# cmbant/getdist

Measured on AMD Instinct MI355X. Metric: 2D KDE densities/sec (triangle, 50 params, 1e+07 samples), higher is better.
Workload: dtype f64

## Files before the change

getdist_amd/_lib.py:

```python

import ctypes as C
import os
import subprocess

import numpy as np

_HERE = os.path.dirname(os.path.abspath(__file__))
LIB_PATH = os.path.join(_HERE, "csrc", "libgdhip.so")

GD_OK, GD_ERR_BADARG, GD_ERR_NOMEM, GD_ERR_HIP, GD_ERR_EMPTY, GD_ERR_SOLVER, GD_ERR_FFT, GD_ERR_NODEVICE, GD_ERR_TIMEOUT = \
    0, -1, -2, -3, -4, -5, -6, -7, -8


class GdhipError(RuntimeError):
    def __init__(self, code, msg):
        super().__init__("libgdhip error %d: %s" % (code, msg))
        self.code = code


class GdhipTimeout(GdhipError):
    """GD_ERR_TIMEOUT: a collective or the communicator set-up gave up waiting for a peer; the library has aborted and dropped
    the communicator, so the ranks renegotiate over the host application's own channel (parallel.init_library_comm)."""


# ... 35 lines not shown
    "gd_kde_lag_sums_2d": (C.c_int, [_p, _i32, _i32, _pd, _pi64, _i32, _pd]),
    "gd_autocov_lags_batch": (C.c_int, [_p, _pi32, _i32, _pd, _i64, _i32, _pd]),
    "gd_kde_lag_sums_batch": (C.c_int, [_p, _pi32, _i32, _pd, _pi64, _i32, _pd]),
    "gd_autocov_lags_range_batch": (C.c_int, [_p, _pi32, _i32, _pd, _i64, _i64, _i64, _i32, _pd]),
    "gd_timer_start": (C.c_int, [_p]),
    "gd_timer_stop_ms": (C.c_int, [_p, _pd]),
    "gd_upload": (C.c_int, [_p, _p, _i64, _i64, _i64, _i64, _p]),
    "gd_num_rows": (C.c_int, [_p, _pi64, _pi64]),
    "gd_column_ptr": (C.c_int, [_p, _i64, C.POINTER(_p)]),
    "gd_weight_stats": (C.c_int, [_p, _i64, _i64, _f64, _pd]),
    "gd_col_stats": (C.c_int, [_p, _i64, _i64, _pd]),
    "gd_cov": (C.c_int, [_p, _pi32, _i32, _i64, _i64, _pd, _pd, _pd, _pd]),
    "gd_quantiles": (C.c_int, [_p, _pi32, _i32, _i64, _i64, _pd, _i32, _pd]),
    "gd_quantiles_mm_probe": (C.c_int, [_p, _pi32, _i32, _i64, _i64, _pd, _i32, _pd, _pd, _pd, _pd, C.POINTER(C.c_int32)]),
    "gd_quantiles_mm": (C.c_int, [_p, _pi32, _i32, _i64, _i64, _pd, _i32, _pd, _pd]),
    "gd_autocov_lags": (C.c_int, [_p, _i32, _f64, _i64, _i32, _pd]),
    "gd_kde_lag_sums": (C.c_int, [_p, _i32, _f64, _pi64, _i32, _pd]),
    "gd_hist1d": (C.c_int, [_p, _pi32, _i32, _pd, _pd, _i32, _pd]),
    "gd_hist1d_dev": (C.c_int, [_p, _pi32, _i32, _pd, _pd, _i32, _p]),
    "gd_bin_indices": (C.c_int, [_p, _i32, _f64, _f64, _i32, _i32, _pi32, _pi64]),
    "gd_prebin": (C.c_int, [_p, _i32, _f64, _f64, _i32, _p]),
    "gd_prebin_batch": (C.c_int, [_p, _pi32, _i32, _pd, _pd, _i32, C.POINTER(_p)]),
    "gd_prebin8_batch": (C.c_int, [_p, _pi32, _i32, _pd, _pd, _i32, C.POINTER(_p), _pi64]),
    "gd_hist2d_prebinned8": (C.c_int, [_p, _i32, C.POINTER(_p), C.POINTER(_p), _p]),
    "gd_prebin8_hist2d": (C.c_int, [_p, _pi32, _i32, _pd, _pd, C.POINTER(_p), _pi64, _i32, C.POINTER(_p), C.POINTER(_p), _p]),
    "gd_hist2d": (C.c_int, [_p, _i32, _pi32, _pi32, _pd, _pd, _pd, _pd, _i32, _p]),
    "gd_hist2d_prebinned": (C.c_int, [_p, _i32, C.POINTER(_p), C.POINTER(_p), _i32, _p]),
    "gd_minmax_affine": (C.c_int, [_p, _i32, _pi32, _pi32, _pd, _pd, _pd]),
    "gd_hist2d_sheared": (C.c_int, [_p, _i32, _pi32, _pi32, _pd, _pd, _pd, _pd, _pd, _pd, _i32, _p]),
    "gd_dct1d": (C.c_int, [_p, _i32, _i32, _pd, _pd]),
    "gd_isj1d": (C.c_int, [_p, _i32, _i32, _pd, _pd, _pd, _pi32]),
    "gd_isj1d_dev": (C.c_int, [_p, _i32, _i32, _p, _pd, _pd, _pi32]),
    "gd_density1d": (C.c_int, [_p, _i32, _i32, _pd, _pd, _pi32, _pi32, _i32, _i32, _pd, _pi32]),
    "gd_density1d_dev": (C.c_int, [_p, _i32, _i32, _p, _pd, _pi32, _pi32, _i32, _i32, _pd, _pi32]),
    "gd_density1d_batch": (C.c_int, [_p, _p, _p, _i32, _pi32, _i32, _pd, _pd, _pd]),
    "gd_kopt2d": (C.c_int, [_p, _i32, _i32, _p, _pd, _pi32, _pd, _pd, _pd]),
    "gd_kopt2d_enqueue": (C.c_int, [_p, _i32, _i32, _p, _pd, _pi32, _pd, _pd, _p, _pi32]),
    "gd_kopt2d_finish": (C.c_int, [_p, _p, _i32, _i32, _p, _pd]),
    "gd_get_h": (C.c_int, [_p, _i32, _pd, _pd, _pd, _pi32, _pd]),
    "gd_density2d": (C.c_int, [_p, _i32, _i32, _p, _pd, _pd, _pd, _pi32, _pi32, _i32, _i32, _p, _pi32]),
    "gd_copy_mark": (C.c_int, [_p, _pi32]),
    "gd_copy_wait": (C.c_int, [_p, _i32]),
    "gd_density2d_enqueue": (C.c_int, [_p, _i32, _i32, _p, _pd, _pd, _pd, _pi32, _pi32, _i32, _i32, _p, _p]),
    "gd_density2d_enqueue_indexed": (C.c_int, [_p, _i32, _i32, _p, _pi32, _pd, _pd, _pd, _pi32, _pi32, _i32, _i32, _p, _p]),
    "gd_attach_samples": (C.c_int, [_p, _p]),
    "gd_clone_samples": (C.c_int, [_p, _p]),
    "gd_bind_thread": (C.c_int, [_p]),
    "gd_contour_levels": (C.c_int, [_p, _i32, _i32, _p, _pd, _i32, _pd, _pi32]),
    "gd_contour_paths": (C.c_int, [_p, _i32, _p, _pi64, _pi32, _pi32, _pd, _pi64, _i64, _pd, _pi64, _i64, _pd, _i32, _p, _p, _pi64,
                                   _pi64, _pi32]),
    "gd_limits1d": (C.c_int, [_p, _i32, _i32, _pd, _pd, _pd, _pd, _i32, _i32, _pd, _pi32]),
    "gd_set_extra_column": (C.c_int, [_p, _i32, _pd]),
    "gd_aux_weights": (C.c_int, [_p, _pd]),
    "gd_col_minmax": (C.c_int, [_p, _pi32, _i32, _i64, _i64, _i32, C.c_double, _pd]),
    "gd_weights_integral": (C.c_int, [_p, _pi32]),
    "gd_thin_rows": (C.c_int, [_p, _i64, _i64, _i64, _i32, _p, _i64, C.POINTER(C.c_int64)]),
    "gd_binary_transitions": (C.c_int, [_p, _pi32, _i32, _p, _i64, _pd, _i32, C.POINTER(C.c_int64)]),
    "gd_thinned_lag_sums": (C.c_int, [_p, _pi32, _i32, _pd, _p, _i64, _i32, _pd]),
    "gd_density2d_masked": (C.c_int, [_p, _i32, _p, C.c_double, C.c_double, C.c_double, _i32, _i32, _i32, _i32, _pd, _pd,
                                      C.POINTER(C.c_ubyte), _p, _pi32]),
    "gd_like_weights": (C.c_int, [_p, _pd, _i32, C.c_double, _pd]),
    "gd_select_weights": (C.c_int, [_p, _i32]),
    "gd_likes1d": (C.c_int, [_p, _i32, _i32, _pd, _pd, _pd, _pd, _pi32, _pi32, _i32, _pd, _pi32]),
    "gd_likes2d": (C.c_int, [_p, _i32, _i32, _p, _p, _pd, _pd, _pd, _pi32, _pi32, _i32, _p, _pi32]),
    "gd_circ_convolve": (C.c_int, [_p, _i32, _i32, _pd, _pd, _pd]),
    "gd_convolve1d_direct": (C.c_int, [_p, _pd, _i64, _pd, _i64, _pd]),
    "gd_autoconvolve": (C.c_int, [_p, _i32, _f64, _i32, _pd, _i64, _i64, _i64, _i32, _pd]),
    "gd_like_stats": (C.c_int, [_p, _i32, _pd]),
    "gd_batch2d_grid_sizes": (C.c_int, [_p, _i32, _pd, _pi32, _i32, _pi32]),
    "gd_density2d_batch": (C.c_int, [_p, _p, _p, _p, _i32, _pd, _pd, _pd, _pi32, _i32, _p, _p, _p, _i64, _pi32, _pd, _pd, _pi32,
                                     _pi32]),
    "gd_comm_unique_id": (C.c_int, [_p]),
    "gd_comm_init": (C.c_int, [_p, _i32, _i32, _p]),
    "gd_comm_info": (C.c_int, [_p, _pi32, _pi32]),
    "gd_comm_destroy": (C.c_int, [_p]),
    "gd_comm_abandon": (C.c_int, [_p]),
    "gd_comm_allgather": (C.c_int, [_p, _pd, _i64, _pd]),
    "gd_comm_allreduce_sum": (C.c_int, [_p, _pd, _i64]),
    "gd_comm_allgather_dev": (C.c_int, [_p, _p, _i64, _p]),
    "gd_comm_allreduce_sum_dev": (C.c_int, [_p, _p, _i64, _p]),
    "gd_batch2d_finish": (C.c_int, [_p]),
    "gd_batch2d_invalidate": (C.c_int, [_p]),
    "gd_batch2d_exchanges": (C.c_int, [_p, C.POINTER(C.c_int64)]),
    "gd_comm_rccl_path": (C.c_int, [C.c_char_p, C.c_int32, C.POINTER(C.c_int32)]),
    "gd_upload_shard": (C.c_int, [_p, _p, _i64, _i64, _i64, _i64, _i64, _p]),
    "gd_comm_share_columns": (C.c_int, [_p, C.POINTER(C.c_int64)]),
    "gd_histnd_batch": (C.c_int, [_p, _i32, _pi32, _pi32, _pd, _pd, _i32, _i32, _i32, _pd, _pd, _pd]),
    "gd_pca_corr": (C.c_int, [_p, _pi32, _i32, _pi32, _pd, _pd, _pd]),
    "gd_pca_project": (C.c_int, [_p, _pi32, _i32, _pi32, _pd, _pd, _pd, _i32, _i32, _pd, _pd, _pd, _pd, _pd, _pd]),
    "gd_mixture_nll": (C.c_int, [_p, _pi32, _i32, _i32, _pd, _pd, _pd, _i64, _i64, _pd]),
    "gd_draw_single_rows": (C.c_int, [_p, C.POINTER(C.c_uint64), _p, _f64, _f64, _i32, _p, _i64, _pi64]),
    "gd_gather_rows": (C.c_int, [_p, _p, _i64, _pi32, _i32, _p]),
    "gd_format_rows": (C.c_int, [_p, _pi32, _i32, _i64, _i64, _p, _i64, _i32, _i32, _i32, _i32, _p, _i64, _pi64]),
    "gd_format_matrix": (C.c_int, [_p, _p, _i64, _i32, _i64, _i64, _i32, _i32, _i32, _i32, _p, _i64, _pi64]),
    "gd_parse_scan": (C.c_int, [_p, _p, _i64, _i32, _pi64, _pi32, _pi64]),
    "gd_parse_rows": (C.c_int, [_p, _p, _i64, _i32, _i64, _i32, _p, _i64, _i64, _p, _i64, _pi64]),
    "gd_expr_eval": (C.c_int, [_p, _pi32, _i32, _pd, _i32, _i32, _i32, _i64, _i64, _p, _pd]),
    "gd_expr_eval_tab": (C.c_int, [_p, _pi32, _i32, _pd, _i32, _i32, _i32, _i64, _i64, _p, _pd, _p, _i32]),
    "gd_upload_device": (C.c_int, [_p, _p, _i32, _i32, _i32, _pi32, _i32, C.POINTER(_p), _i32]),
    "gd_pointer_info": (C.c_int, [_p, _p, _pi32, _pi32]),
    "gd_fetch_device_array": (C.c_int, [_p, _p, _i64, _i64, _i64, _i64, _i32, _p, _pd]),
    "gd_download_samples": (C.c_int, [_p, _pd]),
    "gd_select_samples": (C.c_int, [_p, _p, _pi64]),
    "gd_set_weights": (C.c_int, [_p, _pd]),
    "gd_export_device": (C.c_int, [_p, _p, _pi64]),
    "gd_export_alloc": (C.c_int, [_i32, _i64, C.POINTER(_p)]),
    "gd_export_free": (C.c_int, [_i32, _p]),
    "gd_export_fetch": (C.c_int, [_i32, _p, _p, _i64]),
}

GD_HISTND_MAXD, GD_HISTND_MAX_BINS = 25, 1 << 25
GD_HISTND_H, GD_HISTND_LIKES, GD_HISTND_LMIN = 1, 2, 4
GD_PCA_MAX_PROJ = 448
GD_DRAW_MORE_ROWS = -21
GD_FORMAT_MORE_BYTES = -22
GD_FMT_SRC_WEIGHT, GD_FMT_SRC_ZERO, GD_FMT_SRC_ONE = -1, -2, -3
GD_FMT_MAX_PREC, GD_FMT_MAX_WIDTH = 17, 32
GD_PARSE_NOT_PLAIN = -23
GD_ERR_DECLINED, GD_ERR_OTHER_DEVICE, GD_ERR_NOT_DEVICE = -24, -25, -26
GD_PTR_DEVICE, GD_PTR_PINNED, GD_PTR_MANAGED, GD_PTR_UNKNOWN = 0, 1, 2, 3
GD_PARSE_MAX_LINE = 8192
GD_EX_MAX_CODE, GD_EX_MAX_STACK, GD_EX_MAX_CONST, GD_EX_MAX_COLS = 128, 16, 32, 16
GD_EX_WEIGHT = -1
GD_EX_OPS = ("COL CONST NEG ABS SQRT SQUARE RECIP EXP LOG LOG10 LOG2 SIN COS TAN ATAN TANH NOT ADD SUB MUL DIV POW ATAN2 MIN MAX "
             "LT LE GT GE EQ NE AND OR WHERE").split()
GD_EX_TO_COLUMN, GD_EX_TO_AUXW, GD_EX_TO_HOST_F64, GD_EX_TO_HOST_U8 = 0, 1, 2, 3
GD_TAB_OPS = {"INTERP": 34, "SPLINE1": 35, "SPLINE2": 36}
GD_TAB_MAX_TABLES, GD_TAB_MAX_DOUBLES = 4, 1 << 22
GD_PATHS_XY, GD_PATHS_FLAG, GD_PATHS_LOOPS = 0, 1, 2
PATHS_ALLOC_FN = C.CFUNCTYPE(C.c_void_p, C.c_void_p, _i32, _i64)


class GdExprTable(C.Structure):

    _fields_ = [("kind", _i32), ("deriv", _i32), ("nx", _i32), ("ny", _i32), ("p0", _pd), ("p1", _pd), ("p2", _pd),
                ("left", _f64), ("right", _f64)]


def expr_table_structs(tables):
    arr = (GdExprTable * len(tables))()
    for t, st in zip(tables, arr):
        st.kind, st.deriv, st.nx, st.ny = GD_TAB_OPS[t.kind], t.deriv, t.nx, t.ny
        for name, a in zip(("p0", "p1", "p2"), t.arrays):
            setattr(st, name, _dp(a))
        st.left, st.right = t.left, t.right
    return arr


def format_field_bytes(width, prec):
    return max(int(width), int(prec) + 8) + 1


def skipped_text_bytes(f, skiprows):
    start = 0
    for _ in range(int(skiprows or 0)):
        line = f.readline()
        if not line:
            break
        if b"\r" in line.replace(b"\r\n", b"") or b"\0" in line or not line.isascii():
            return None
        start += len(line)
    return start


class GdDevPart(C.Structure):

    _fields_ = [("base", _p), ("rows", _i64), ("cols", _i64), ("row_stride", _i64), ("col_stride", _i64), ("weights", _p),
                ("w_stride", _i64)]


class GdSelection(C.Structure):

    _fields_ = [("row_kind", _i32), ("flags", _i32), ("lo", _i64), ("hi", _i64), ("rows", _p), ("K", _i64), ("thr", _f64),
                ("keep", _p), ("m", _i32), ("append_kind", _i32), ("append_slot", _i32), ("weight_kind", _i32),
                ("append_host", _p), ("new_weights", _p)]


class GdExport(C.Structure):

    _fields_ = [("row_kind", _i32), ("flags", _i32), ("lo", _i64), ("hi", _i64), ("rows", _p), ("K", _i64), ("thr", _f64),
                ("mask_col", _i32), ("m", _i32), ("cols", _p), ("base", _p), ("rows_capacity", _i64), ("row_stride", _i64),
                ("col_stride", _i64), ("dtype", _i32), ("reserved", _i32), ("consumer_stream", _p)]


GD_EXP_ROWS_COLUMN_NZ = 5

GD_SEL_ALL, GD_SEL_RANGE, GD_SEL_MASK_U8, GD_SEL_WEIGHT_GT, GD_SEL_ROWS_I32 = range(5)
GD_SEL_W_KEEP, GD_SEL_W_UNIT, GD_SEL_W_REPLACE = range(3)
GD_SEL_APPEND_NONE, GD_SEL_APPEND_HOST, GD_SEL_APPEND_SLOT = range(3)
GD_SEL_ROWS_ON_DEVICE = 1
GD_SEL_TILE = 1024

_lib = None


def load_library():
    global _lib
    if _lib is None:
        if not os.path.exists(LIB_PATH):
            raise ImportError("libgdhip.so is not built: run `python -c 'import __graft_entry__ as g; g.build()'` "
                              "or getdist_amd/csrc/build.sh (there is no CPU fallback)")
        lib = C.CDLL(LIB_PATH)
        for name, (res, args) in SIGNATURES.items():
            fn = getattr(lib, name)
            fn.restype = res
            fn.argtypes = args
        _lib = lib
    return _lib


def _dp(a):
    return a.ctypes.data_as(_pd)


def _ip(a):
    return a.ctypes.data_as(_pi32)


def _f64arr(a):
    return np.ascontiguousarray(a, dtype=np.float64)


def _i32arr(a):
    return np.ascontiguousarray(a, dtype=np.int32)


class DevBuf:

    def __init__(self, ctx, nbytes):
        self.ctx = ctx
        self.nbytes = int(nbytes)
        self.ptr, self.capacity = ctx._take_block(self.nbytes)

    def free(self):
        if self.ptr and self.ctx.h:
            self.ctx._give_block(self.ptr, self.capacity)
        self.ptr = None

    def __del__(self):
        try:
            self.free()
        except Exception:
            pass

    def to_host(self, shape, dtype=np.float64, offset_bytes=0, pinned=False):
        out = self.ctx.pinned_array(shape, dtype) if pinned else np.empty(shape, dtype=dtype)
        self.ctx._check(self.ctx.lib.gd_memcpy_d2h(self.ctx.h, out.ctypes.data, self.ptr + offset_bytes, out.nbytes))
        return out

    def to_host_async(self, shape, dtype=np.float64):
        out = self.ctx.pinned_array(shape, dtype)
        self.ctx._check(self.ctx.lib.gd_memcpy_d2h_async(self.ctx.h, out.ctypes.data, self.ptr, out.nbytes))
        return out

    def from_host(self, arr, offset_bytes=0):
        arr = np.ascontiguousarray(arr)
        self.ctx._check(self.ctx.lib.gd_memcpy_h2d(self.ctx.h, self.ptr + offset_bytes, arr.ctypes.data, arr.nbytes))


class ExportBlock:

    def __init__(self, device, nbytes):
        self.lib, self.device, self.nbytes = load_library(), int(device), int(nbytes)
        p = _p()
        rc = self.lib.gd_export_alloc(self.device, self.nbytes, C.byref(p))
        if rc == GD_ERR_NOMEM:
            raise MemoryError("no room for a device array of %d bytes on device %d" % (self.nbytes, self.device))
        if rc != 0:
            raise GdhipError(rc, "gd_export_alloc(%d bytes) failed" % self.nbytes)
        self.ptr = p.value

    def fetch(self, out):
        rc = self.lib.gd_export_fetch(self.device, out.ctypes.data, self.ptr, out.nbytes)
        if rc != 0:
            raise GdhipError(rc, "gd_export_fetch failed")
        return out

    def __del__(self):
        try:
            if self.ptr:
                self.lib.gd_export_free(self.device, self.ptr)
            self.ptr = None
        except Exception:
            pass


class Context:

    def __init__(self, device=0):
        self.lib = load_library()
        self.h = None
# ... 396 lines not shown
            ex.row_kind, ex.mask_col = GD_EXP_ROWS_COLUMN_NZ, int(rows[1])
        elif kind != "all":
            raise ValueError("unknown row selection %r" % (kind,))
        if cols is not None:
            c = _i32arr(cols).ravel()
            alive.append(c)
            ex.cols, ex.m = c.ctypes.data, c.size
        if dest is not None:
            if dest.ndim != 2 or dest.shape[1] != (1 if cols is None else len(c)):
                raise ValueError("the destination must be 2-D with one column per exported column")
            ex.base, ex.rows_capacity = dest.ptr or None, dest.shape[0]
            ex.row_stride, ex.col_stride, ex.dtype = dest.strides[0], dest.strides[1], int(dest.dtype)
        ex.consumer_stream = stream
        count = C.c_int64()
        rc = self.lib.gd_export_device(self.h, C.byref(ex), C.byref(count))
        if rc == GD_DRAW_MORE_ROWS:
            if dest is None:
                return int(count.value)
            raise ValueError("the destination has %d rows, %d are selected" % (dest.shape[0], count.value))
        if rc == GD_ERR_DECLINED:
            raise ValueError("out= must be plain device memory with non-negative strides (%s)" % self.lib.gd_last_error(self.h).decode())
        if rc == GD_ERR_BADARG:
            raise ValueError(self.lib.gd_last_error(self.h).decode())
        self._served(rc, [] if dest is None else [dest])
        return int(count.value)

    def set_weights(self, w):
        if w is not None:
            w = _f64arr(w)
            if w.shape != (self.N,):
                raise ValueError("weights must have one entry per sample row")
        self._check(self.lib.gd_set_weights(self.h, None if w is None else _dp(w)))
        self._keep = None
        self.weighted = w is not None

    def bind_thread(self):
        self._check(self.lib.gd_bind_thread(self.h))

    def column_ptr(self, j):
        p = _p()
        self._check(self.lib.gd_column_ptr(self.h, int(j), C.byref(p)))
        return p.value

    def weight_stats(self, lo=0, hi=None, thresh=np.inf):
        out = np.zeros(4)
        self._check(self.lib.gd_weight_stats(self.h, lo, self.N if hi is None else hi, float(thresh), _dp(out)))
        return dict(norm=out[0], max_w=out[1], sum_w2=out[2], n_above=out[3])

    def col_stats(self, lo=0, hi=None):
        out = np.zeros((self.n, 4))
        self._check(self.lib.gd_col_stats(self.h, lo, self.N if hi is None else hi, _dp(out)))
        return out

    def cov(self, cols=None, lo=0, hi=None, minmax=False):
        cols = _i32arr(np.arange(self.n) if cols is None else cols)
        m = len(cols)
        means, cov, norm = np.zeros(m), np.zeros((m, m)), C.c_double()
        mm = np.zeros((m, 2)) if minmax else None
        self._check(self.lib.gd_cov(self.h, _ip(cols), m, lo, self.N if hi is None else hi, _dp(means), _dp(cov),
                                    C.byref(norm), None if mm is None else _dp(mm)))
        return (means, cov, norm.value, mm) if minmax else (means, cov, norm.value)

    def quantiles(self, cols, targets, lo=0, hi=None, minmax=None):
        cols = _i32arr(cols)
        targets = _f64arr(targets).reshape(len(cols), -1)
        out = np.zeros_like(targets)
        mm = None if minmax is None else _f64arr(minmax).reshape(len(cols), 2)
        self._check(self.lib.gd_quantiles_mm(self.h, _ip(cols), len(cols), lo, self.N if hi is None else hi, _dp(targets),
                                             targets.shape[1], None if mm is None else _dp(mm), _dp(out)))
        return out

    def quantiles_probe(self, cols, targets, minmax, means):
        cols = _i32arr(cols)
        targets = _f64arr(targets).reshape(len(cols), -1)
        out = np.zeros_like(targets)
        mm = _f64arr(minmax).reshape(len(cols), 2)
        means = _f64arr(means)
        probe = np.zeros((len(cols), 8))
        done = C.c_int32(0)
        self._check(self.lib.gd_quantiles_mm_probe(self.h, _ip(cols), len(cols), 0, self.N, _dp(targets), targets.shape[1], _dp(mm),
                                                   _dp(out), _dp(means), _dp(probe), C.byref(done)))
        return out, (probe if done.value else None)

    def autocov_lags(self, col, mean, k0, nlags):
        out = np.zeros(nlags)
        self._check(self.lib.gd_autocov_lags(self.h, int(col), float(mean), int(k0), int(nlags), _dp(out)))
        return out

    def kde_lag_sums(self, col, inv4s2, lags):
        lags = np.ascontiguousarray(lags, dtype=np.int64)
        out = np.zeros(len(lags))
        self._check(self.lib.gd_kde_lag_sums(self.h, int(col), float(inv4s2), lags.ctypes.data_as(_pi64), len(lags),
                                             _dp(out)))
        return out

    def hist1d(self, cols, binmin, width, F):
        cols, binmin, width = _i32arr(cols), _f64arr(binmin), _f64arr(width)
        out = np.zeros((len(cols), F))
        self._check(self.lib.gd_hist1d(self.h, _ip(cols), len(cols), _dp(binmin), _dp(width), int(F), _dp(out)))
        return out

    def bin_indices(self, col, binmin, width, F, round_half=True):
        idx = np.zeros(self.N, dtype=np.int32)
        bad = C.c_int64()
        self._check(self.lib.gd_bin_indices(self.h, int(col), float(binmin), float(width), int(bool(round_half)), int(F),
                                            _ip(idx), C.byref(bad)))
        return idx, bad.value

    def prebin(self, col, binmin, width, F, buf=None):
        buf = buf or self.alloc(self.N * 2 + 64)
        self._check(self.lib.gd_prebin(self.h, int(col), float(binmin), float(width), int(F), buf.ptr))
        return buf

    def prebin_batch(self, cols, binmin, width, F, bufs):
        cols, binmin, width = _i32arr(cols), _f64arr(binmin), _f64arr(width)
        arr = (_p * len(cols))(*[b.ptr for b in bufs])
        self._check(self.lib.gd_prebin_batch(self.h, _ip(cols), len(cols), _dp(binmin), _dp(width), int(F), arr))

    def prebin8_batch(self, cols, binmin, width, F, bufs):
        cols, binmin, width = _i32arr(cols), _f64arr(binmin), _f64arr(width)
        arr = (_p * len(cols))(*[b.ptr for b in bufs])
        bad = np.zeros(len(cols), dtype=np.int64)
        self._check(self.lib.gd_prebin8_batch(self.h, _ip(cols), len(cols), _dp(binmin), _dp(width), int(F), arr,
                                              bad.ctypes.data_as(_pi64)))
        return bad

    def hist2d_prebinned8(self, idx_x, idx_y, out=None):
        B = len(idx_x)
        out = out or self.alloc(B * 65536 * 8)
        if isinstance(idx_x, np.ndarray):
            px, py = np.ascontiguousarray(idx_x, dtype=np.uint64), np.ascontiguousarray(idx_y, dtype=np.uint64)
            ax, ay = px.ctypes.data_as(C.POINTER(_p)), py.ctypes.data_as(C.POINTER(_p))
        else:
            ax = (_p * B)(*[b.ptr for b in idx_x])
            ay = (_p * B)(*[b.ptr for b in idx_y])
        self._check(self.lib.gd_hist2d_prebinned8(self.h, B, ax, ay, out.ptr))
        return out

    def hist2d(self, colx, coly, bx, wx, by, wy, F, out=None):
        colx, coly = _i32arr(colx), _i32arr(coly)
        B = len(colx)
        out = out or self.alloc(B * F * F * 8)
        bx, wx, by, wy = _f64arr(bx), _f64arr(wx), _f64arr(by), _f64arr(wy)
        self._check(self.lib.gd_hist2d(self.h, B, _ip(colx), _ip(coly), _dp(bx), _dp(wx), _dp(by), _dp(wy), int(F),
                                       out.ptr))
        return out

    def hist2d_prebinned(self, idx_x, idx_y, F, out=None):
        B = len(idx_x)
        out = out or self.alloc(B * F * F * 8)
        ax = (_p * B)(*[b.ptr for b in idx_x])
        ay = (_p * B)(*[b.ptr for b in idx_y])
        self._check(self.lib.gd_hist2d_prebinned(self.h, B, ax, ay, int(F), out.ptr))
        return out

    def minmax_affine(self, coli, colj, a, b):
        coli, colj, a, b = _i32arr(coli), _i32arr(colj), _f64arr(a), _f64arr(b)
        out = np.zeros((len(coli), 2))
        self._check(self.lib.gd_minmax_affine(self.h, len(coli), _ip(coli), _ip(colj), _dp(a), _dp(b), _dp(out)))
        return out

    def hist2d_sheared(self, coli, colj, r0, r1, xmin, dx, ymin, dy, F, out=None):
        coli, colj = _i32arr(coli), _i32arr(colj)
        B = len(coli)
        out = out or self.alloc(B * F * F * 8)
        arrs = [_f64arr(v) for v in (r0, r1, xmin, dx, ymin, dy)]
# ... 616 lines not shown
```

getdist_amd/csrc/batch2d.hip:

```cpp
#include "batch1d.hpp"
#include "batch2d.hpp"
#include "ctx.hpp"

namespace {

gd_ctx* C(void* h) { return (gd_ctx*)h; }

const gdb::Ops kOps = {
     [](void* h) { return gd_bind_thread(C(h)); },
     [](void* h, int64_t* N, int64_t* n) { return gd_num_rows(C(h), N, n); },
    [](void* h, int32_t* hw) {
        gd_ctx* c = C(h);
        *hw = c->w == nullptr ? 0 : ((!c->w8 && !c->w_integral && c->w_sum > 1e-200 && c->w_sum < 1e200) ? 2 : 1);
        return 0;
    },
     [](void* h, int64_t bytes, void** out) { return gd_dev_alloc(C(h), bytes, out); },
     [](void* h, void* p) { return gd_dev_free(C(h), p); },
    [](void* h, const int32_t* cols, int32_t ncols, const double* binmin, const double* width, int32_t F, void* const* d_idx,
       int64_t* bad) { return gd_prebin8_batch(C(h), cols, ncols, binmin, width, F, d_idx, bad); },
    [](void* h, int32_t B, const void* const* ix, const void* const* iy, void* d_hist) {
        return gd_hist2d_prebinned8(C(h), B, ix, iy, d_hist);
    },
    [](void* h, const int32_t* cols, int32_t ncols, const double* binmin, const double* width, void* const* d_idx, int64_t* bad,
       int32_t B, const void* const* ix, const void* const* iy, void* d_hist) {
        return gd_prebin8_hist2d(C(h), cols, ncols, binmin, width, d_idx, bad, B, ix, iy, d_hist);
    },
    [](void* h, int32_t col, double binmin, double width, int32_t F, void* d_idx) {
        return gd_prebin(C(h), col, binmin, width, F, d_idx);
    },
    [](void* h, int32_t B, const void* const* ix, const void* const* iy, int32_t F, void* d_hist) {
        return gd_hist2d_prebinned(C(h), B, ix, iy, F, d_hist);
    },
    [](void* h, int32_t B, const int32_t* ci, const int32_t* cj, const double* a, const double* b, double* out) {
        return gd_minmax_affine(C(h), B, ci, cj, a, b, out);
    },
    [](void* h, int32_t B, const int32_t* ci, const int32_t* cj, const double* r0, const double* r1, const double* xmin,
       const double* dx, const double* ymin, const double* dy, int32_t F, void* d_hist) {
        return gd_hist2d_sheared(C(h), B, ci, cj, r0, r1, xmin, dx, ymin, dy, F, d_hist);
    },
    [](void* h, int32_t B, int32_t F, const void* d_hist, const double* neff, const int32_t* do_corr, const double* fallback_t,
       const double* corr, double* out) { return gd_kopt2d(C(h), B, F, d_hist, neff, do_corr, fallback_t, corr, out); },
    [](void* h, void* d_dst, int64_t dst_first, const void* d_src, const int32_t* index, int32_t count, int64_t item_bytes) {
        return gd_gather_items(C(h), (char*)d_dst + dst_first * item_bytes, d_src, index, count, item_bytes);
    },
    [](void* h, int32_t B, int32_t F, const void* d_hist, const int32_t* hist_index, const double* rx, const double* ry,
       const double* corr, const int32_t* winw, const int32_t* flags, int32_t bco, int32_t mbc, void* d_P, int32_t* status_pinned) {
        return gd_density2d_enqueue_indexed(C(h), B, F, d_hist, hist_index, rx, ry, corr, winw, flags, bco, mbc, d_P, status_pinned);
    },
     [](void* h, void* dst, const void* d_src, int64_t bytes) { return gd_memcpy_d2h_async(C(h), dst, d_src, bytes); },
     [](void* h, int32_t* token) { return gd_copy_mark(C(h), token); },
    [](void* h, int32_t token) {
        if (!gd_ctx_alive(C(h))) return 0;
        const int rc = gd_copy_wait(C(h), token);
        return rc == GD_ERR_BADARG ? 0 : rc;
    },
     [](void* h) { return gd_ctx_alive(C(h)) ? gd_copy_sync(C(h)) : 0; },
    [](void* h, int32_t B, int32_t F, const void* d_P, const double* contours, int32_t nc, double* out, int32_t* status) {
        return gd_contour_levels(C(h), B, F, d_P, contours, nc, out, status);
    },
    [](void* h, const int32_t* cols, int32_t ncols, const double* means, int64_t k0, int32_t nlags, double* out) {
        return gd_autocov_lags_batch(C(h), cols, ncols, means, k0, nlags, out);
    },
    [](void* h, const int32_t* cols, int32_t ncols, const double* inv4s2, const int64_t* lags, int32_t nlags, double* out) {
        return gd_kde_lag_sums_batch(C(h), cols, ncols, inv4s2, lags, nlags, out);
    },
    [](void* h, int32_t col, double inv4s2, const int64_t* lags, int32_t nlags, double* out) {
        return gd_kde_lag_sums(C(h), col, inv4s2, lags, nlags, out);
    },
     [](void* h) { return gd_last_error(C(h)); },
    [](void* h, void** aux) {
        gd_ctx* a = nullptr;
        int rc = gd_create(C(h)->device, &a);
        if (rc == 0) rc = gd_attach_samples(a, C(h));
        if (rc == 0) rc = gd_stream_priority(a, 1);
        if (rc) {
            if (a) gd_destroy(a);
            return gd_fail(C(h), rc, "could not create the third context of a batched call");
        }
        *aux = a;
        return 0;
    },
    [](void* aux) {
        gd_destroy(C(aux));
        return 0;
    },
    [](void* h, int32_t B, int32_t F, const void* d_hist, const double* neff, const int32_t* do_corr, const double* fallback_t,
       const double* corr, void* d_rows, int32_t* ticket) {
        return gd_kopt2d_enqueue(C(h), B, F, d_hist, neff, do_corr, fallback_t, corr, d_rows, ticket);
    },
    [](void* h, void* stage_a_h, int32_t ticket, int32_t B, void* d_rows, double* out) {
        return gd_kopt2d_finish(C(h), C(stage_a_h), ticket, B, d_rows, out);
    },
     [](void* h) { return C(h)->comm ? C(h)->comm_world : 0; },
     [](void* h, double* inout, int64_t count) { return gd_comm_allreduce_sum(C(h), inout, count); },
     [](void* ctx, int level) { return gd_stream_priority(C(ctx), level); },
    [](void* h, const int32_t* cols, int32_t ncols, const double* binmin, const double* width, int32_t F, void* const* d_idx) {
        return gd_prebin_batch(C(h), cols, ncols, binmin, width, F, d_idx);
    },
};

const gdb::Ops1D kOps1D = {
    [](void* h, const int32_t* cols, int32_t ncols, const double* binmin, const double* width, int32_t F, void* d_hist) {
        return gd_hist1d_dev(C(h), cols, ncols, binmin, width, F, d_hist);
    },
    [](void* h, int32_t B, int32_t F, const void* d_hist, const double* neff, double* hfrac, int32_t* status) {
        return gd_isj1d_dev(C(h), B, F, d_hist, neff, hfrac, status);
    },
    [](void* h, int32_t B, int32_t F, const void* d_hist, const double* smooth, const int32_t* winw, const int32_t* flags,
       int32_t bco, int32_t mbc, double* P_out, int32_t* status) {
        return gd_density1d_dev(C(h), B, F, d_hist, smooth, winw, flags, bco, mbc, P_out, status);
    },
    [](void* h, void* dst, const void* d_src, int64_t bytes) {
        const int rc = gd_fetch(C(h), dst, d_src, (size_t)bytes);
        return rc ? rc : gd_stream_sync(C(h));
    },
};

void release_state(gd_ctx* ctx, bool destroy) {
    gdb::State* st = (gdb::State*)ctx->batch_state;
    if (!st) return;
    gdb::release_all(*st, kOps, ctx);
    if (destroy) {
        delete st;
        ctx->batch_state = nullptr;
    }
}

gdb::State& state_of(gd_ctx* ctx) {
    if (!ctx->batch_state) {
        ctx->batch_state = new gdb::State();
        ctx->batch_state_release = release_state;
    }
    return *(gdb::State*)ctx->batch_state;
}

}

extern "C" {

int gd_batch2d_grid_sizes(const gd_batch2d_settings* settings, int32_t n, const double* corr, const int32_t* pairs, int32_t P,
                          int32_t* F_out) {
    if (!settings || !corr || (!pairs && P > 0) || (!F_out && P > 0) || n <= 0 || P < 0) return GD_ERR_BADARG;
    for (int k = 0; k < 2 * P; ++k)
        if (pairs[k] < 0 || pairs[k] >= n) return GD_ERR_BADARG;
    gdb::PairScalars ps;
    gdb::pair_scalars(*settings, n, corr, pairs, P, ps);
    for (int k = 0; k < P; ++k) F_out[k] = ps.F[k];
    return GD_OK;
}

int gd_density2d_batch(gd_ctx* ctx, gd_ctx* twin, const gd_batch2d_settings* settings, gd_param2d* params, int32_t n,
                       const double* corr, const double* cov, const double* lag_probe, const int32_t* pairs, int32_t P,
                       gd_neff_exchange_fn exchange, void* exchange_user, void* grids_pinned, int64_t grids_doubles,
                       int32_t* status_pinned, double* meta, double* levels, int32_t* level_status, int32_t* tokens_out2) {
    GD_REQUIRE(ctx && settings && params && corr && cov && tokens_out2 && n > 0 && P >= 0, "bad argument");
    GD_REQUIRE(P == 0 || (pairs && grids_pinned && status_pinned && meta), "bad argument");
    GD_REQUIRE(ctx->cols, "no samples uploaded");
    GD_REQUIRE(!twin || (twin != ctx && twin->cols == ctx->cols), "the second context must be attached to the first (gd_attach_samples)");
    GD_REQUIRE(ctx->w_sel == 0, "auxiliary weights are selected");
    GD_REQUIRE(!settings->want_levels || (settings->contours && settings->ncontours > 0 && levels && level_status), "contour levels requested without room for them");
    GD_HIP(hipSetDevice(ctx->device));
    int rc;
    try {
        gdb::Call call(state_of(ctx), kOps, ctx, twin, *settings, params, n, corr, cov, lag_probe, pairs, P, exchange, exchange_user,
                       (double*)grids_pinned, grids_doubles, status_pinned, meta, levels, level_status);
        rc = call.run(tokens_out2);
        if (rc) ctx->err = call.err;
    } catch (const std::exception& e) {
        rc = gd_fail(ctx, GD_ERR_NOMEM, "gd_density2d_batch: %s", e.what());
    }
    return rc;
}

int gd_density1d_batch(gd_ctx* ctx, const gd_density1d_settings* settings, gd_param2d* params, int32_t n, const int32_t* cols,
                       int32_t B, double* P_out, double* hist_out, double* meta) {
    GD_REQUIRE(ctx && settings && params && cols && P_out && meta && n > 0 && B > 0, "bad argument");
    GD_REQUIRE(ctx->cols, "no samples uploaded");
    GD_REQUIRE(ctx->w_sel == 0, "auxiliary weights are selected");
    GD_HIP(hipSetDevice(ctx->device));
    int rc;
    try {
        std::string err;
        rc = gdb::density1d_batch(state_of(ctx), kOps, kOps1D, ctx, *settings, params, n, cols, B, P_out, hist_out, meta, &err);
        if (rc) ctx->err = err;
    } catch (const std::exception& e) {
        rc = gd_fail(ctx, GD_ERR_NOMEM, "gd_density1d_batch: %s", e.what());
    }
    return rc;
}

int gd_batch2d_finish(gd_ctx* ctx) {
    GD_REQUIRE(ctx, "null context");
    if (!ctx->batch_state) return GD_OK;
    GD_HIP(hipSetDevice(ctx->device));
    return gdb::finish_all(*(gdb::State*)ctx->batch_state, kOps, ctx);
}

int gd_batch2d_exchanges(gd_ctx* ctx, int64_t* count_out) {
    GD_REQUIRE(ctx && count_out, "null argument");
    *count_out = 0;
    if (ctx->batch_state) {
        gdb::State& st = *(gdb::State*)ctx->batch_state;
        std::lock_guard<std::mutex> g(st.mu);
        *count_out = st.exchanges_entered;
    }
    return GD_OK;
}

int gd_batch2d_invalidate(gd_ctx* ctx) {
    GD_REQUIRE(ctx, "null context");
    if (!ctx->batch_state) return GD_OK;
    gdb::invalidate_index_columns(*(gdb::State*)ctx->batch_state);
    return GD_OK;
}

}
```

getdist_amd/csrc/batch2d.hpp:

```cpp
#pragma once
#include <math.h>
#include <stdint.h>
#include <stdio.h>
#include <stdlib.h>
#include <string.h>
#include <time.h>

#include <algorithm>
#include <atomic>
#include <chrono>
#include <condition_variable>
#include <deque>
#include <functional>
#include <future>
#include <map>
#include <mutex>
#include <string>
#include <thread>
#include <vector>

#include "../../include/gdhip.h"

namespace gdb {

// ... 47 lines not shown
static inline double py_pow(double x, double y) {
    volatile double e = y;
    return pow(x, e);
}
static inline double np_minimum(double a, double b) { return (a < b || isnan(a)) ? a : b; }
static inline double np_maximum(double a, double b) { return (a > b || isnan(a)) ? a : b; }
static inline double np_sign(double x) { return isnan(x) ? x : (x > 0 ? 1.0 : (x < 0 ? -1.0 : 0.0)); }

static inline int frame_size(int n) {
    long long best = 1LL << 40;
    const int odd[5] = {1, 3, 5, 9, 15};
    for (int a = 4; a < 28; ++a)
        for (int q = 0; q < 5; ++q) {
            const long long v = (1LL << a) * odd[q];
            if (v >= n && v < best) best = v;
        }
    return (int)best;
}

static inline bool chol_shear(double c00, double c10, double c11, double S[4], double r[2]) {
    if (!(c00 > 0)) return false;
    const double l00 = sqrt(c00);
    const double l10 = c10 * (1.0 / l00);
    const double d = c11 - l10 * l10;
    if (!(d > 0)) return false;
    const double l11 = sqrt(d);
    double i00, i10, i11;
    if (fabs(l10) > fabs(l00)) {
        const double l = l00 * (1.0 / l10);
        const double u11 = 0.0 - l * l11;
        i10 = 1.0 * (1.0 / u11);
        i00 = (0.0 - l11 * i10) * (1.0 / l10);
        i11 = (0.0 - l * 1.0) * (1.0 / u11);
    } else {
        const double l = l10 * (1.0 / l00);
        i00 = 1.0 * (1.0 / l00);
        i10 = (0.0 - l * 1.0) * (1.0 / l11);
        i11 = 1.0 * (1.0 / l11);
    }
    S[0] = l00 * i00, S[1] = 0.0 * i00, S[2] = l10 * i00, S[3] = l11 * i00;
    r[0] = i10 / i00, r[1] = i11 / i00;
    return true;
}

struct PairScalars {
    std::vector<int32_t> jx, jy, F, warn;
    std::vector<int64_t> nbin2D;
    std::vector<double> actual, corr;
};

static inline void pair_scalars(const gd_batch2d_settings& s, int n, const double* corrmat, const int32_t* pairs, int P,
                                PairScalars& ps) {
    ps.jx.resize(P), ps.jy.resize(P), ps.F.resize(P), ps.warn.assign(P, 0), ps.nbin2D.resize(P), ps.actual.resize(P),
        ps.corr.resize(P);
    const int base_F = s.fine_bins_2D;
    for (int k = 0; k < P; ++k) {
        const int a = pairs[2 * k], b = pairs[2 * k + 1];
        ps.jx[k] = a, ps.jy[k] = b;
        const double actual = corrmat[(size_t)b * n + a];
        double c = actual;
        if (fabs(fabs(c) - 1.0) <= 1e-8) {
            ps.warn[k] |= 1;
            c = np_sign(c) * s.max_corr_2D;
        }
        if (fabs(c) < 0.1) c = 0.0;
        const double m = np_minimum(s.max_corr_2D, fabs(c));
        const double angle_scale = np_maximum(0.2, sqrt(1 - m * m));
        ps.nbin2D[k] = (int64_t)nearbyint((double)s.num_bins_2D / angle_scale);
        const int64_t scaled = 192 * (int64_t)(3 / angle_scale) / 3;
        ps.F[k] = (c != 0 && base_F < scaled && (int64_t)(1 / angle_scale) > 1) ? (int32_t)scaled : base_F;
        ps.actual[k] = actual, ps.corr[k] = c;
    }
}

static inline void bin_edges(const gd_param2d& p, double* binmin, double* binmax) {
    const double border = (p.range_max - p.range_min) * 0.1;
    double lo = np_minimum(p.param_min, p.range_min);
    if (!p.has_limits_bot) lo = lo - border;
    double hi = np_maximum(p.param_max, p.range_max);
    if (!p.has_limits_top) hi = hi + border;
    *binmin = lo, *binmax = hi;
}

struct NeffInput {
    int64_t N;
    double norm, sum_w2;
};

static inline int neff_from_lags(const NeffInput& in, int64_t maxoff, double min_corr, const double* sums, int nseed_tail,
                                 const std::function<int(int64_t, double*)>& lag_sum, double* neff_out) {
    const int64_t N = in.N;
    if (maxoff > N / 10) maxoff = N / 10;
    const int64_t uncorr_len = N / 2;
    int64_t nav = 0;
    for (int64_t k = uncorr_len; k < uncorr_len + 5; ++k) nav += N - k;
    double s5 = 0.0;
    for (int q = 0; q < 5; ++q) s5 += sums[q];
    const double uncorr_term = s5 / (double)nav;
    const double n = (double)N;
    std::map<int64_t, double> cache;
    for (int q = 0; q < nseed_tail; ++q) cache[q + 1] = sums[5 + q];
    int rc = 0;
    auto corr_k = [&](int64_t k) -> double {
        auto it = cache.find(k);
        double v;
        if (it == cache.end()) {
            v = NAN;
            const int e = lag_sum(k, &v);
            if (e) rc = e;
            cache[k] = v;
        } else {
            v = it->second;
        }
        return v - (n - (double)k) * uncorr_term;
    };
    const double corr0 = in.sum_w2;
    const double threshold = min_corr * corr0;
    const double c1 = corr_k(1);
    double Nn;
    if (c1 < threshold) {
        Nn = corr0;
    } else {
        const double c2 = corr_k(2);
        if (c2 > threshold) {
            int64_t max_k = maxoff;
            while (max_k > 10) {
                if (corr_k(max_k / 3) >= threshold) break;
                max_k /= 3;
            }
            const int64_t step_size = max_k < 20 ? 1 : max_k / 10;
            double cum_sum = c1 + c2;
            for (int64_t k = 3; k < maxoff + 1; k += step_size) {
                const double test_val = corr_k(k);
                if (test_val < threshold) break;
                cum_sum += k > 3 ? test_val * (double)step_size : (test_val * (double)step_size) / 2;
            }
            Nn = corr0 + 2 * cum_sum;
        } else {
            Nn = corr0 + 2 * c1;
        }
    }
    if (rc) return rc;
    *neff_out = py_pow(in.norm, 2.0) / Nn;
    return 0;
}

struct Plan {
    std::vector<int8_t> branch;
    std::vector<uint8_t> has_limits;
    std::vector<double> rangex, rangey, ratio, neff, fallback_t;
    std::vector<int32_t> si, sj;
    std::vector<uint8_t> swap, has_imin, has_imax;
    std::vector<double> imin, imax, S, r;
};

static inline bool has_limits(const gd_param2d& p) { return p.has_limits_bot || p.has_limits_top; }

static inline int make_plan(const gd_batch2d_settings& s, const gd_param2d* par, int n, const double* cov,
                            const PairScalars& ps, const std::vector<double>& rngx, const std::vector<double>& rngy,
                            double min_corr, Plan& pl, std::string& err) {
    const int P = (int)ps.jx.size();
    pl.branch.resize(P), pl.has_limits.resize(P), pl.rangex = rngx, pl.rangey = rngy, pl.ratio.resize(P);
    pl.neff.assign(P, NAN), pl.fallback_t.assign(P, NAN);
    pl.si.assign(P, -1), pl.sj.assign(P, -1), pl.swap.assign(P, 0), pl.has_imin.assign(P, 0), pl.has_imax.assign(P, 0);
    pl.imin.assign(P, NAN), pl.imax.assign(P, NAN), pl.S.assign((size_t)4 * P, NAN), pl.r.assign((size_t)2 * P, NAN);
    for (int k = 0; k < P; ++k) {
        const gd_param2d &px = par[ps.jx[k]], &py = par[ps.jy[k]];
        const bool limx = has_limits(px), limy = has_limits(py);
        pl.has_limits[k] = limx || limy;
        const bool do_correlated = !limx || !limy;
        const double c = ps.actual[k], absc = fabs(c);
        const bool is_A = (min_corr < absc) && (absc <= s.max_corr_2D) && do_correlated;
        const bool is_B = !is_A && ((absc > s.max_corr_2D) || (!do_correlated && (c > 0.8)));
        pl.branch[k] = is_A ? 0 : (is_B ? 1 : 2);
        pl.ratio[k] = np_minimum(py.sigma_range / rngy[k], px.sigma_range / rngx[k]);
        if (!is_A) continue;
        int i = ps.jx[k], j = ps.jy[k];
        if (px.has_limits_bot) pl.has_imin[k] = 1, pl.imin[k] = px.range_min;
        if (px.has_limits_top) pl.has_imax[k] = 1, pl.imax[k] = px.range_max;
        if (limy) {
            std::swap(i, j);
            pl.swap[k] = 1;
            if (py.has_limits_bot) pl.has_imin[k] = 1, pl.imin[k] = py.range_min;
            if (py.has_limits_top) pl.has_imax[k] = 1, pl.imax[k] = py.range_max;
        }
        pl.si[k] = i, pl.sj[k] = j;
        if (!chol_shear(cov[(size_t)i * n + i], cov[(size_t)j * n + i], cov[(size_t)j * n + j], &pl.S[(size_t)4 * k],
                        &pl.r[(size_t)2 * k])) {
            err = "Matrix is not positive definite";
            return GD_ERR_BADARG;
        }
    }
    return 0;
}

static inline void fill_plan(const gd_param2d* par, const PairScalars& ps, Plan& pl, const double* pair_neff = nullptr) {
    const int P = (int)ps.jx.size();
    for (int k = 0; k < P; ++k) {
        pl.neff[k] = pair_neff ? pair_neff[k] : np_minimum(par[ps.jx[k]].neff, par[ps.jy[k]].neff);
        if (pl.branch[k] == 2) pl.fallback_t[k] = py_pow(pl.ratio[k] / py_pow(pl.neff[k], 1.0 / 6), 2.0);
    }
}

struct IdxCol {
    void* ptr = nullptr;
    double binmin = NAN, width = NAN;
    bool valid = false;
};

struct Pending {
    std::vector<void*> blocks;
    int32_t tok_main = -1, tok_twin = -1;
    void* twin = nullptr;
    bool live = false;
};

struct State {
    std::mutex mu;
    std::vector<std::pair<void*, int64_t>> free_blocks;
    std::map<void*, int64_t> capacity;
    int64_t cached_bytes = 0;
    std::map<std::tuple<int, int, int>, IdxCol> idx;
    Pending prev;
    void* aux = nullptr;
    void* aux2 = nullptr;
    int64_t exchanges_entered = 0;
    static constexpr int64_t kCacheLimit = 16LL << 30;
};

struct Pool {
    State& st;
    const Ops& ops;
    void* h;
    void* take(int64_t bytes, int* rc) {
        {
            std::lock_guard<std::mutex> g(st.mu);
            int best = -1;
            for (size_t k = 0; k < st.free_blocks.size(); ++k) {
                const int64_t cap = st.free_blocks[k].second;
                if (cap >= bytes && cap <= 2 * bytes + (1 << 20) && (best < 0 || cap < st.free_blocks[best].second)) best = (int)k;
            }
            if (best >= 0) {
                void* p = st.free_blocks[best].first;
                st.cached_bytes -= st.free_blocks[best].second;
                st.free_blocks.erase(st.free_blocks.begin() + best);
                return p;
            }
        }
        void* p = nullptr;
        int e = ops.dev_alloc(h, bytes, &p);
        if (e == GD_ERR_NOMEM) {
            drop_cached();
            e = ops.dev_alloc(h, bytes, &p);
        }
        if (e) {
            *rc = e;
            return nullptr;
        }
        std::lock_guard<std::mutex> g(st.mu);
        st.capacity[p] = bytes;
        return p;
    }
    void give(void* p) {
        if (!p) return;
        std::unique_lock<std::mutex> g(st.mu);
        const int64_t cap = st.capacity[p];
        if (st.cached_bytes + cap > State::kCacheLimit) {
            st.capacity.erase(p);
            g.unlock();
            ops.dev_free(h, p);
            return;
        }
        st.free_blocks.emplace_back(p, cap);
        st.cached_bytes += cap;
    }
    void drop_cached() {
        std::vector<std::pair<void*, int64_t>> blocks;
        {
            std::lock_guard<std::mutex> g(st.mu);
            blocks.swap(st.free_blocks);
            st.cached_bytes = 0;
            for (auto& b : blocks) st.capacity.erase(b.first);
        }
        for (auto& b : blocks) ops.dev_free(h, b.first);
    }
};

static inline int complete_pending(State& st, const Ops& ops, void* h, Pending& pd) {
    if (!pd.live) return 0;
    int rc = 0;
    if (pd.tok_main >= 0) rc = ops.copy_wait(h, pd.tok_main);
    if (!rc && pd.twin && pd.tok_twin >= 0) rc = ops.copy_wait(pd.twin, pd.tok_twin);
    Pool pool{st, ops, h};
    for (void* p : pd.blocks) pool.give(p);
    pd.blocks.clear();
    pd.live = false;
    return rc;
}

static inline int finish_all(State& st, const Ops& ops, void* h) { return complete_pending(st, ops, h, st.prev); }

static inline void invalidate_index_columns(State& st) {
    std::lock_guard<std::mutex> g(st.mu);
    for (auto& kv : st.idx) kv.second.valid = false;
}

static inline void release_all(State& st, const Ops& ops, void* h) {
    finish_all(st, ops, h);
// ... 105 lines not shown
        size_t part = std::max<size_t>((size_t)s_kopt_split_min(), (total + want - 1) / want);
        size_t align = 256;
        if (const char* e = getenv("GDHIP_KOPT_PART_ALIGN")) align = (size_t)std::max(0, atoi(e));
        if (align > 1 && F == 256 && part > align) part = std::max<size_t>(align, (part + align / 2 - 1) / align * align);
        return part;
    }
    static size_t first_part_size(size_t part) {
        if (const char* e = getenv("GDHIP_KOPT_FIRST_PART")) {
            const size_t f = (size_t)std::max(0, atoi(e));
            if (f > 0 && f < part) return f;
        }
        return part;
    }
    static int shear_hold_us() {
        const char* e = getenv("GDHIP_BATCH_SHEAR_HOLD_US");
        return e ? atoi(e) : 0;
    }
    int join_shear(bool release = false) {
        if (release) first_part_done.store(1);
        std::lock_guard<std::mutex> g(shear_mu);
        if (shear_joined.load()) return 0;
        const int e = shear_future.valid() ? shear_future.get() : 0;
        shear_joined.store(true);
        mark("shear: joined");
        return e;
    }
    int64_t grid_off = 0;
    int status_at = 0;
    int batch_no = 0;
    std::vector<void*> conv_ctxs;
    std::vector<int> side_classes;
    std::vector<int> order;

    std::mutex tl_mu;
    std::vector<std::pair<double, std::string>> tl;
    bool tl_on = getenv("GDHIP_BATCH_LOG") != nullptr;
    static double now_ms() {
        timespec ts;
        clock_gettime(CLOCK_MONOTONIC, &ts);
        return ts.tv_sec * 1e3 + ts.tv_nsec * 1e-6;
    }
    void mark(const char* what, int a = -1, int b = -1) {
        if (!tl_on) return;
        char buf[160];
        if (a >= 0 && b >= 0)
            snprintf(buf, sizeof buf, "%s (%d, %d)", what, a, b);
        else if (a >= 0)
            snprintf(buf, sizeof buf, "%s (%d)", what, a);
        else
            snprintf(buf, sizeof buf, "%s", what);
        std::lock_guard<std::mutex> g(tl_mu);
        tl.emplace_back(now_ms(), buf);
    }
    void dump_timeline() {
        if (!tl_on || tl.empty()) return;
        std::sort(tl.begin(), tl.end());
        fprintf(stderr, "---- gd_density2d_batch host timeline (ms)\n");
        for (auto& e : tl) fprintf(stderr, "%9.3f  %s\n", e.first - tl[0].first, e.second.c_str());
    }

    std::mutex err_mu;
    int fail(int code, const std::string& msg) {
        std::lock_guard<std::mutex> g(err_mu);
        if (err.empty()) err = msg;
        return code;
    }
    int dev_fail(int code, void* ctx) {
        const char* m = ops.last_error(ctx);
        return fail(code, m && *m ? m : "device call failed");
    }
#define GDB_DEV(ctx_, call_)                       \
    do {                                           \
        const int rc__ = (call_);                  \
        if (rc__) return dev_fail(rc__, (ctx_));   \
    } while (0)
#define GDB_TRY(call_)            \
    do {                          \
        const int rc__ = (call_); \
        if (rc__) return rc__;    \
    } while (0)

    double* M(int k) { return meta + (size_t)k * GD_BATCH2D_META; }

    int neff_batch(const std::vector<int>& js, bool owned_only, double min_corr = 0.05) {
        std::vector<int32_t> todo;
        for (int j : js)
            if (isnan(par[j].neff) && (!owned_only || (par[j].owned & 1))) todo.push_back(j);
        if (todo.empty()) return 0;
        mark("neff: start", (int)todo.size());
        if (s.uncorrelated_sampler) {
            for (int j : todo) par[j].neff = py_pow(s.norm, 2.0) / s.sum_w2;
            return 0;
        }
        const int m = (int)todo.size();
        const int64_t max_off = N / 10;
        const int nl = (int)std::min<int64_t>(8, max_off + 1);
        std::vector<double> lag0((size_t)m * nl);
        bool have = lag_probe != nullptr && nl == 8;
        if (have)
            for (int row = 0; row < m && have; ++row)
                for (int k = 0; k < nl; ++k) {
                    lag0[(size_t)row * nl + k] = lag_probe[(size_t)todo[row] * 8 + k];
                    if (isnan(lag0[(size_t)row * nl + k])) have = false;
                }
        if (!have) {
            std::vector<double> means(m);
            for (int row = 0; row < m; ++row) means[row] = par[todo[row]].mean;
            GDB_DEV(h, ops.autocov_lags_batch(h, todo.data(), m, means.data(), 0, nl, lag0.data()));
        }
        std::vector<double> kstd(m), inv4s2(m);
        std::vector<int64_t> maxoffs(m);
        bool all_uncorrelated_at_lag_1 = true;
        for (int row = 0; row < m; ++row) {
            const gd_param2d& p = par[todo[row]];
            double c[8];
            for (int k = 0; k < nl; ++k) c[k] = lag0[(size_t)row * nl + k] / (double)(N - k) / p.var;
            int first_below = -1;
            for (int k = 0; k < nl; ++k)
                if (!(c[k] > min_corr * c[0])) {
                    first_below = k;
                    break;
                }
            if (first_below != 1) all_uncorrelated_at_lag_1 = false;
            double corrlen;
            if (first_below >= 0) {
                double sum = 0.0;
                for (int k = 1; k < first_below; ++k) sum += c[k];
                corrlen = c[0] + 2 * sum;
            } else if (nl == max_off + 1) {
                corrlen = c[0];
            } else {
                char buf[160];
                snprintf(buf, sizeof buf, "column %d: the chain's correlation outlasts the 8-lag probe (getCorrelationLength's long route)",
                         (int)todo[row]);
                return fail(GD_BATCH2D_NEED_NEFF, buf);
            }
            const double sr = p.sigma_range;
            kstd[row] = ((isnan(sr) || sr == 0.0) ? p.err : sr) * 0.2;
            inv4s2[row] = 1.0 / (4 * py_pow(kstd[row], 2.0));
            maxoffs[row] = (int64_t)(corrlen * 1.5) + 4;
        }
        std::vector<int64_t> lags;
        const int64_t uncorr_len = N / 2;
        for (int64_t k = uncorr_len; k < uncorr_len + 5; ++k) lags.push_back(k);
        int ntail = 0;
        for (int64_t k : {1, 2})
            if (k <= N / 10 && (k == 1 || !all_uncorrelated_at_lag_1)) lags.push_back(k), ++ntail;
        const int L = (int)lags.size();
        std::vector<double> sums((size_t)m * L);
        mark("neff: probe done");
        if (hold_neff_for_binning) {
            const auto t0 = std::chrono::steady_clock::now();
            while (!bin_launching.load() && std::chrono::steady_clock::now() - t0 < std::chrono::milliseconds(2)) std::this_thread::yield();
            int hold_us = 120;
            if (const char* e = getenv("GDHIP_BATCH_NEFF_HOLD_US")) hold_us = atoi(e);
            if (bin_launching.load()) std::this_thread::sleep_for(std::chrono::microseconds(hold_us));
            mark("neff: binning chain enqueued");
        }
        GDB_DEV(h, ops.kde_lag_sums_batch(h, todo.data(), m, inv4s2.data(), lags.data(), L, sums.data()));
        mark("neff: lag sums done");
        const NeffInput in{N, s.norm, s.sum_w2};
        for (int row = 0; row < m; ++row) {
            const int col = todo[row];
            const double i4 = inv4s2[row];
            auto lag_sum = [&](int64_t k, double* out) -> int { return ops.kde_lag_sums(h, col, i4, &k, 1, out); };
            double v = NAN;
            const int e = neff_from_lags(in, maxoffs[row], min_corr, &sums[(size_t)row * L], ntail, lag_sum, &v);
            if (e) return dev_fail(e, h);
            par[col].neff = v;
        }
        return 0;
    }

    int neff_exchange(bool* exchanged) {
        if (exchange && !*exchanged) {
            *exchanged = true;
            std::vector<double> v(n);
            for (int j = 0; j < n; ++j) v[j] = par[j].neff;
            if (exchange(exchange_user, v.data(), n)) return fail(GD_ERR_HIP, "N_eff exchange failed");
            for (int j = 0; j < n; ++j)
                if (isnan(par[j].neff)) par[j].neff = v[j];
        } else if (!exchange && s.comm_exchange && !*exchanged) {
            *exchanged = true;
            if (!ops.comm_world || ops.comm_world(h) < 1) return fail(GD_ERR_BADARG, "comm_exchange without a communicator (gd_comm_init)");
            {
                std::lock_guard<std::mutex> g(st.mu);
                ++st.exchanges_entered;
            }
            std::vector<double> v(n, 0.0);
            for (int j = 0; j < n; ++j)
                if ((par[j].owned & 1) && !isnan(par[j].neff)) v[j] = par[j].neff;
            GDB_DEV(h, ops.comm_allreduce_sum(h, v.data(), n));
            for (int j = 0; j < n; ++j)
                if (isnan(par[j].neff) && v[j] > 0) par[j].neff = v[j];
        }
        return 0;
    }
    int neff_complete(bool* exchanged) {
        const int rc = neff_exchange(exchanged);
        if (rc || s.pair_neff) return rc;
        return neff_batch(used, false);
    }

    int index_column16(void* ctx, int j, int F, void** out) {
        const double fw = (bmax[j] - bmin[j]) / (F - 1);
        IdxCol c;
        {
            std::lock_guard<std::mutex> g(st.mu);
            c = st.idx[std::make_tuple(j, F, 2)];
        }
        if (!(c.valid && c.binmin == bmin[j] && c.width == fw)) {
            if (!c.ptr) {
                int rc = 0;
                c.ptr = pool.take(N * 2 + 64, &rc);
                if (!c.ptr) return dev_fail(rc, h);
            }
            GDB_DEV(ctx, ops.prebin(ctx, j, bmin[j], fw, F, c.ptr));
            c.binmin = bmin[j], c.width = fw, c.valid = true;
            std::lock_guard<std::mutex> g(st.mu);
            st.idx[std::make_tuple(j, F, 2)] = c;
        }
        *out = c.ptr;
        return 0;
    }

    int index_columns16(void* ctx, const std::vector<int>& cols, int F) {
        if (!ops.prebin_batch) return 0;
        std::vector<int32_t> todo;
        std::vector<double> b0, w;
        std::vector<void*> bufs;
        for (int j : cols) {
            const double fw = (bmax[j] - bmin[j]) / (F - 1);
            IdxCol c;
            {
                std::lock_guard<std::mutex> g(st.mu);
                c = st.idx[std::make_tuple(j, F, 2)];
            }
            if (c.valid && c.binmin == bmin[j] && c.width == fw) continue;
            if (!c.ptr) {
                int rc = 0;
                c.ptr = pool.take(N * 2 + 64, &rc);
                if (!c.ptr) return dev_fail(rc, h);
                std::lock_guard<std::mutex> g(st.mu);
                st.idx[std::make_tuple(j, F, 2)] = c;
            }
            todo.push_back(j), b0.push_back(bmin[j]), w.push_back(fw), bufs.push_back(c.ptr);
        }
        if (todo.size() < 2) return 0;
        GDB_DEV(ctx, ops.prebin_batch(ctx, todo.data(), (int)todo.size(), b0.data(), w.data(), F, bufs.data()));
        std::lock_guard<std::mutex> g(st.mu);
        for (size_t q = 0; q < todo.size(); ++q) {
            IdxCol& c = st.idx[std::make_tuple((int)todo[q], F, 2)];
            c.binmin = b0[q], c.width = w[q], c.valid = true;
        }
        return 0;
    }

    int main_class() const {
        int best = F_list.empty() ? 0 : F_list[0];
        for (int F : F_list)
            if (classes.at(F).size() > classes.at(best).size()) best = F;
        return best;
    }
    int binning(void* ctx, int part = 0) {
        const int main_F = main_class();
        for (int F : F_list) {
            if ((part == 1 && F != main_F) || (part == 2 && F == main_F)) continue;
            const std::vector<int>& members = classes.at(F);
            const int B = (int)members.size();
            int rc = 0;
            if (F == 256 && (unit_weights || byte_index_weights) && B >= 64) {
                std::vector<int> cols;
                std::vector<char> seen(n, 0);
                for (int k : members)
                    if (!seen[ps.jx[k]]) seen[ps.jx[k]] = 1, cols.push_back(ps.jx[k]);
                for (int k : members)
                    if (!seen[ps.jy[k]]) seen[ps.jy[k]] = 1, cols.push_back(ps.jy[k]);
                std::vector<int32_t> todo;
                std::vector<double> b0, w;
                std::vector<void*> bufs;
                {
                    std::lock_guard<std::mutex> g(st.mu);
                    for (int j : cols) {
                        const double fw = (bmax[j] - bmin[j]) / 255;
                        IdxCol& c = st.idx[std::make_tuple(j, 256, 1)];
                        if (c.valid && c.binmin == bmin[j] && c.width == fw) continue;
                        todo.push_back(j), b0.push_back(bmin[j]), w.push_back(fw), bufs.push_back(c.ptr);
                    }
                }
                for (size_t q = 0; q < todo.size(); ++q)
                    if (!bufs[q]) {
                        bufs[q] = pool.take(N + 64, &rc);
                        if (!bufs[q]) return dev_fail(rc, h);
                        std::lock_guard<std::mutex> g(st.mu);
                        IdxCol& c = st.idx[std::make_tuple((int)todo[q], 256, 1)];
                        c.ptr = bufs[q], c.valid = false;
                    }
                std::vector<const void*> ix(B), iy(B);
                {
                    std::lock_guard<std::mutex> g(st.mu);
                    for (int q = 0; q < B; ++q) {
                        ix[q] = st.idx[std::make_tuple((int)ps.jx[members[q]], 256, 1)].ptr;
                        iy[q] = st.idx[std::make_tuple((int)ps.jy[members[q]], 256, 1)].ptr;
                    }
                }
                void* d = pool.take((int64_t)B * 65536 * 8, &rc);
                if (!d) return dev_fail(rc, h);
                std::vector<int64_t> bad(todo.size() + 1, 0);
                mark("binning: prebin8 + hist2d launch", (int)todo.size(), B);
                bin_launching.store(1);
                const int B1 = (F == main_F && bins_first_rows > 0 && bins_first_rows < B) ? bins_first_rows : B;
                int e = ops.prebin8_hist2d(ctx, todo.data(), (int)todo.size(), b0.data(), w.data(), bufs.data(), bad.data(), B1,
                                           ix.data(), iy.data(), d);
                mark("binning: prebin8 + hist2d done", B1);
                if (e == 0 || e == GD_ERR_SOLVER) {
                    std::lock_guard<std::mutex> g(st.mu);
                    for (size_t q = 0; q < todo.size(); ++q) {
                        IdxCol& c = st.idx[std::make_tuple((int)todo[q], 256, 1)];
                        c.binmin = b0[q], c.width = w[q], c.valid = bad[q] == 0;
                    }
                }
                bool published = false;
                if (e == 0 && B1 < B) {
                    {
                        std::lock_guard<std::mutex> g(enq_mu);
                        hists[F] = d;
                    }
                    published = true;
                    bins_first_done.store(1);
                    e = ops.hist2d_prebinned8(ctx, B - B1, ix.data() + B1, iy.data() + B1, (char*)d + (int64_t)B1 * 65536 * 8);
                    mark("binning: the other rows done", B - B1);
                    if (e == 0) continue;
                }
                if (e == 0) {
                    std::lock_guard<std::mutex> g(enq_mu);
                    hists[F] = d;
                    continue;
                }
                if (published) {
                    std::lock_guard<std::mutex> g(enq_mu);
                    hists.erase(F);
                    bin_stale.push_back(d);
                } else {
                    pool.give(d);
                }
                if (e != GD_ERR_SOLVER) return dev_fail(e, ctx);
            }
            bin_launching.store(1);
            {
                std::vector<int> cols;
                std::vector<char> seen(n, 0);
                for (int k : members) {
                    if (!seen[ps.jx[k]]) seen[ps.jx[k]] = 1, cols.push_back(ps.jx[k]);
                    if (!seen[ps.jy[k]]) seen[ps.jy[k]] = 1, cols.push_back(ps.jy[k]);
// ... 886 lines not shown
```

getdist_amd/csrc/binning.hip:

```cpp
#include "ctx.hpp"

#include <array>
#include <map>

#define LDS_HIST_BYTES (128 * 1024)

struct BinDiv {
    double binmin, width, rcp;
};
__device__ __forceinline__ BinDiv make_bindiv(double binmin, double width) {
    BinDiv d;
    d.binmin = binmin, d.width = width;
    const unsigned long long mant = (unsigned long long)__double_as_longlong(width) & 0xFFFFFFFFFFFFFull;
    d.rcp = (mant == 0xFFFFFFFFFFFFFull) ? 0.0 : 1.0 / width;
    return d;
}
__device__ __forceinline__ double bin_quotient(double x, const BinDiv& d) {
    const double n = x - d.binmin;
    double q = n * d.rcp;
    double r = fma(-q, d.width, n);
    q = fma(r, d.rcp, q);
    r = fma(-q, d.width, n);
    q = fma(r, d.rcp, q);
    if (!(fabs(q) < 1e300) || d.rcp == 0.0) q = n / d.width;
// ... 1248 lines not shown
int gd_hist2d_prebinned(gd_ctx* ctx, int32_t B, const void* const* d_idx_x, const void* const* d_idx_y, int32_t F,
                        void* d_hist) {
    GD_REQUIRE(ctx && d_idx_x && d_idx_y && d_hist && B > 0, "bad argument");
    GD_REQUIRE(ctx->cols, "no samples uploaded");
    GD_REQUIRE(F >= 2 && F <= 4096, "fine_bins_2D out of range");
    std::vector<Hist2DPair> hp((size_t)B);
    for (int b = 0; b < B; ++b) {
        Hist2DPair& p = hp[b];
        memset(&p, 0, sizeof p);
        p.ix = (const unsigned short*)d_idx_x[b];
        p.iy = (const unsigned short*)d_idx_y[b];
        GD_REQUIRE(p.ix && p.iy, "null index column");
    }
    {
        int R16 = LDS_HIST_BYTES / (F * 2);
        if (R16 > F) R16 = F;
        const int nstripes16 = (F + R16 - 1) / R16;
        if (!ctx->w && (int64_t)B * nstripes16 < ctx->cu_count && !getenv("GDHIP_NO_U16_CHUNKS")) {
            const int R = R16, nstripes = nstripes16;
            const int nchunks = pick_chunks(ctx, (int64_t)B * nstripes, ctx->N);
            const int units = (B * nchunks + 7) / 8 * 8;
            const int64_t nblocks = (int64_t)units * nstripes;
            const int nwords = (R * F + 1) / 2;
            ScratchPlan sp;
            auto d_pairs = sp.take<Hist2DPair>(B);
            auto d_flags = sp.take<int>(B);
            auto d_part = sp.tail<unsigned int>((int64_t)B * nchunks * nstripes * nwords);
            GD_TRY(sp.get2(ctx));
            GD_TRY(gd_h2d(ctx, d_pairs, hp.data(), (size_t)B * sizeof(Hist2DPair)));
            GD_HIP(hipMemsetAsync(d_flags, 0, (size_t)B * 4, ctx->stream));
            GD_HIP(hipFuncSetAttribute((const void*)k_hist2d_u16_chunks, hipFuncAttributeMaxDynamicSharedMemorySize, LDS_HIST_BYTES));
            k_hist2d_u16_chunks<<<(unsigned)nblocks, 1024, (size_t)nwords * 4, ctx->stream>>>(d_pairs, B, ctx->N, F, R, nstripes, nchunks,
                                                                                              d_part, d_flags);
            GD_KERNEL_CHECK();
            k_p16_reduce<<<dim3((unsigned)((nwords + 255) / 256), nstripes, B), 256, 0, ctx->stream>>>(d_part, F, R, nstripes, nchunks, (double*)d_hist);
            GD_KERNEL_CHECK();
            std::vector<int> hf((size_t)B);
            GD_TRY(gd_fetch(ctx, hf.data(), d_flags, (size_t)B * 4));
            GD_TRY(gd_stream_sync(ctx));
            std::vector<int> flagged;
            for (int b = 0; b < B; ++b)
                if (hf[b]) flagged.push_back(b);
            int rc = GD_OK;
            if (!flagged.empty()) {
                const int nf = (int)flagged.size();
                std::vector<Hist2DPair> sub((size_t)nf);
                for (int q = 0; q < nf; ++q) sub[q] = hp[flagged[q]];
                double* tmp = nullptr;
                GD_HIP(hipMalloc((void**)&tmp, (size_t)nf * F * F * 8));
                rc = launch_hist2d<2>(ctx, nf, sub, F, tmp);
                for (int q = 0; q < nf && rc == GD_OK; ++q)
                    if (hipMemcpyAsync((double*)d_hist + (int64_t)flagged[q] * F * F, tmp + (int64_t)q * F * F, (size_t)F * F * 8,
                                       hipMemcpyDeviceToDevice, ctx->stream) != hipSuccess)
                        rc = gd_fail(ctx, GD_ERR_HIP, "copy of redone histogram failed");
                (void)hipStreamSynchronize(ctx->stream);
                (void)hipFree(tmp);
            }
            return rc;
        }
        if ((ctx->w && !ctx->w8) || (int64_t)B * nstripes16 < ctx->cu_count)
            return launch_hist2d<2>(ctx, B, hp, F, (double*)d_hist);
    }
    std::vector<int> flagged;
    int rc = launch_hist2d_u16(ctx, B, hp, F, (double*)d_hist, flagged);
    if (rc) return rc;
    if (!flagged.empty()) {
        const int nf = (int)flagged.size();
        std::vector<Hist2DPair> sub((size_t)nf);
        for (int q = 0; q < nf; ++q) sub[q] = hp[flagged[q]];
        double* tmp = nullptr;
        GD_HIP(hipMalloc((void**)&tmp, (size_t)nf * F * F * 8));
        rc = launch_hist2d<2>(ctx, nf, sub, F, tmp);
        if (rc == GD_OK)
            for (int q = 0; q < nf && rc == GD_OK; ++q)
                if (hipMemcpyAsync((double*)d_hist + (int64_t)flagged[q] * F * F, tmp + (int64_t)q * F * F, (size_t)F * F * 8,
                                   hipMemcpyDeviceToDevice, ctx->stream) != hipSuccess)
                    rc = gd_fail(ctx, GD_ERR_HIP, "copy of redone histogram failed");
        (void)hipStreamSynchronize(ctx->stream);
        (void)hipFree(tmp);
    }
    return rc;
}

int gd_prebin8_batch(gd_ctx* ctx, const int32_t* cols, int32_t ncols, const double* binmin, const double* width, int32_t F,
                     void* const* d_idx_out, int64_t* bad_out) {
    GD_REQUIRE(ctx && cols && binmin && width && d_idx_out && bad_out && ncols > 0, "bad argument");
    GD_REQUIRE(ctx->cols, "no samples uploaded");
    GD_REQUIRE(F >= 2 && F <= 256, "byte indices need fine_bins_2D <= 256");
    for (int c = 0; c < ncols; ++c) GD_REQUIRE(cols[c] >= 0 && cols[c] < ctx->n + GD_EXTRA_COLS && d_idx_out[c], "bad column");
    const BucketRoute R = bucket_route(ctx, cols, ncols, binmin, width, d_idx_out);
    std::vector<PrebinCol8> hc;
    std::vector<int> fp_of((size_t)ncols, -1);
    for (int c = 0; c < ncols; ++c) {
        if (R.slot_of[c] >= 0) continue;
        PrebinCol8 r;
        r.x = ctx->cols + (int64_t)cols[c] * ctx->ld;
        r.idx = (unsigned char*)d_idx_out[c];
        r.binmin = binmin[c];
        r.width = width[c];
        fp_of[c] = (int)hc.size();
        hc.push_back(r);
    }
    const int nfp = (int)hc.size();
    BucketRouteLayout L(ctx, R);
    ScratchPlan sp;
    auto d_c = sp.take<PrebinCol8>(nfp);
    auto d_bad = sp.take<unsigned long long>(nfp);
    auto d_route = sp.tail<char>(L.sp.bytes());
    GD_TRY(sp.get2(ctx));
    L.sp.place(d_route);
    if (nfp) {
        GD_TRY(gd_h2d(ctx, d_c, hc.data(), (size_t)nfp * sizeof(PrebinCol8)));
        GD_HIP(hipMemsetAsync(d_bad, 0, (size_t)nfp * 8, ctx->stream));
        int nblk = (int)((ctx->N / 8 + 255) / 256);
        if (nblk > 2 * ctx->cu_count) nblk = 2 * ctx->cu_count;
        if (nblk < 1) nblk = 1;
        k_prebin8_batch<<<dim3(nblk, nfp), 256, 0, ctx->stream>>>(d_c, ctx->N, F, d_bad);
        GD_KERNEL_CHECK();
    }
    unsigned long long* d_bad_bq = nullptr;
    if (!R.recs.empty()) GD_TRY(bucket_route_launch<true>(ctx, R, L, F, &d_bad_bq));
    std::vector<unsigned long long> hb((size_t)nfp), hq(R.recs.size());
    if (nfp) GD_TRY(gd_fetch(ctx, hb.data(), d_bad, (size_t)nfp * 8));
    if (!R.recs.empty()) GD_TRY(gd_fetch(ctx, hq.data(), d_bad_bq, hq.size() * 8));
    GD_TRY(gd_stream_sync(ctx));
    for (int c = 0; c < ncols; ++c) bad_out[c] = (int64_t)(R.slot_of[c] >= 0 ? hq[R.slot_of[c]] : hb[fp_of[c]]);
    return GD_OK;
}

#define WP_TILE 4096
#ifndef WS
#define WS 16
#endif
#define WR (256 / WS)
#define WPG (WS / 4)
#define WXB 8
struct WKey {
    const unsigned char* iy;
    unsigned char* ij_perm;
    unsigned long long* wq_perm;
    int64_t npad;
    int x_first, x_count;
};
struct WX {
    const unsigned char* ix;
    unsigned char* ix_perm;
};

__global__ void __launch_bounds__(256) k_wpart_count(const WKey* __restrict__ keys, int64_t N, int ntiles, int* __restrict__ counts) {
    __shared__ int c[WS];
    const WKey K = keys[blockIdx.y];
    if (threadIdx.x < WS) c[threadIdx.x] = 0;
    __syncthreads();
    const int64_t base = (int64_t)blockIdx.x * WP_TILE;
    for (int e = threadIdx.x * 16; e < WP_TILE; e += 256 * 16) {
        const int64_t r = base + e;
        if (r + 16 <= N) {
            const uint4 v = gload_u4(K.iy + r);
            const unsigned wd[4] = {v.x, v.y, v.z, v.w};
#pragma unroll
            for (int q = 0; q < 16; ++q) atomicAdd(&c[((wd[q >> 2] >> (8 * (q & 3))) & 0xff) / WR], 1);
        } else {
            for (int q = 0; q < 16 && r + q < N; ++q) atomicAdd(&c[K.iy[r + q] / WR], 1);
        }
    }
    __syncthreads();
    if (threadIdx.x < WS) counts[((int64_t)blockIdx.y * ntiles + blockIdx.x) * WS + threadIdx.x] = c[threadIdx.x];
}

#define WLPS (1024 / WS)
__global__ void __launch_bounds__(1024) k_wpart_scan(const int* __restrict__ counts, int ntiles, int64_t* __restrict__ offsets,
                                                     int64_t* __restrict__ starts) {
    __shared__ int64_t tot[WS];
    __shared__ int64_t chunk_base[WS][WLPS + 1];
    const int s = threadIdx.x / WLPS, lane = threadIdx.x % WLPS;
    const int* c = counts + (int64_t)blockIdx.x * ntiles * WS;
    const int per = (ntiles + WLPS - 1) / WLPS;
    const int t0 = lane * per, t1 = min(ntiles, t0 + per);
    int64_t mine = 0;
    for (int i = t0; i < t1; ++i) mine += (c[(int64_t)i * WS + s] + 15) & ~15;
    chunk_base[s][lane] = mine;
    __syncthreads();
    if (lane == 0) {
        int64_t run = 0;
        for (int l = 0; l < WLPS; ++l) {
            const int64_t v = chunk_base[s][l];
            chunk_base[s][l] = run;
            run += v;
        }
        tot[s] = run;
    }
    __syncthreads();
    int64_t off = 0;
    for (int q = 0; q < s; ++q) off += tot[q];
    if (lane == 0) {
        starts[(int64_t)blockIdx.x * (WS + 1) + s] = off;
        if (s == WS - 1) starts[(int64_t)blockIdx.x * (WS + 1) + WS] = off + tot[s];
    }
    off += chunk_base[s][lane];
    int64_t* o = offsets + (int64_t)blockIdx.x * ntiles * WS;
    for (int i = t0; i < t1; ++i) {
        o[(int64_t)i * WS + s] = off;
        off += (c[(int64_t)i * WS + s] + 15) & ~15;
    }
}

__global__ void __launch_bounds__(1024) k_wpart_scatter(const WKey* __restrict__ keys, const WX* __restrict__ xs, const double* __restrict__ w,
                                                        int64_t N, int ntiles, const int* __restrict__ counts,
                                                        const int64_t* __restrict__ offsets, double wscale) {
// ... 501 lines not shown
```

getdist_amd/csrc/ctx.hpp:

```cpp
#pragma once
#include <hip/hip_runtime.h>
#include <stdint.h>
#include <stdio.h>
#include <string.h>

#include <map>
#include <memory>
#include <mutex>
#include <set>
#include <string>
#include <atomic>
#include <type_traits>
#include <vector>

#include "../../include/gdhip.h"
#include "scratchplan.hpp"

struct FftPlanCache;

struct BucketCols {
    std::mutex mu;
    unsigned short* buf = nullptr;
    int64_t n = 0, ld = 0;
    bool tried = false;
// ... 15 lines not shown
    hipEvent_t ev0 = nullptr, ev1 = nullptr;
    int cu_count = 256;
    std::string err;
    double* cols = nullptr;
    double* w = nullptr;
    bool w_integral = false;
    unsigned char* w8 = nullptr;
    unsigned char* w8_main = nullptr;
    double* like_w = nullptr;
    double* w_main = nullptr;
    bool w_main_integral = false;
    double w_sum = 0, w_main_sum = 0;
    int w_sel = 0;
    bool borrowed = false;
    long long* wcum = nullptr;
    std::shared_ptr<BucketCols> bq;
    int64_t N = 0, n = 0, ld = 0;
    void* scratch = nullptr;
    int64_t scratch_bytes = 0;
    void* scratch2 = nullptr;
    int64_t scratch2_bytes = 0;
    void* gather_index = nullptr;
    int64_t gather_index_bytes = 0;
    FftPlanCache* fft = nullptr;
    std::map<int, double*> dctmat;
    std::map<int, void*> fft_tw;
    struct StageSlot {
        void* host = nullptr;
        size_t cap = 0;
        hipEvent_t ev = nullptr;
        bool used = false;
        bool own = false;
    };
    static constexpr size_t kStageBytes = 64u << 10;
    void* stage_block = nullptr;
    static constexpr int kCopyMarks = 16;
    hipEvent_t copy_marks[kCopyMarks] = {};
    int copy_mark_next = 0;
    static constexpr int kStageSlots = 32;
    StageSlot stage[kStageSlots];
    int stage_next = 0;
    struct Fetch {
        void* dst;
        size_t off, bytes;
    };
    static constexpr size_t kFetchBytes = 4u << 20, kFetchMax = 1u << 20;
    void* fetch_block = nullptr;
    size_t fetch_off = 0;
    std::vector<Fetch> fetch_pending;
    static constexpr int kKoptEvents = 32;
    hipEvent_t kopt_evs[kKoptEvents] = {};
    int kopt_ev_next = 0;
    void* comm = nullptr;
    int comm_world = 0, comm_rank = 0;
    void* comm_buf = nullptr;
    size_t comm_buf_bytes = 0;
    std::atomic<int> comm_abandon_gen{0};
    int comm_completed = 0;
    void* batch_state = nullptr;
    void (*batch_state_release)(gd_ctx*, bool destroy) = nullptr;
};

int gd_stage_h2d(gd_ctx* ctx, void* d_dst, const void* src, size_t bytes);
int gd_h2d(gd_ctx* ctx, void* d_dst, const void* src, size_t bytes);

int gd_fft_r2c_2d(gd_ctx* ctx, int n0, int n1, int batch, const double* d_in, double2* d_out);
int gd_fft_c2r_2d(gd_ctx* ctx, int n0, int n1, int batch, double2* d_in, double* d_out);
void gd_fft_cache_destroy(gd_ctx* ctx);

int gd_fetch(gd_ctx* ctx, void* host_dst, const void* d_src, size_t bytes);
int gd_fetch_pinned(gd_ctx* ctx, void* pinned_dst, const void* d_src, size_t bytes);
int gd_stream_sync(gd_ctx* ctx);

int gd_upload_release(gd_ctx* ctx);
void gd_upload_install(gd_ctx* ctx, double* cols, double* w, unsigned char* w8, bool integral, double wsum, int64_t N, int64_t n,
                       int64_t ld);
int gd_upload_weight_flags(gd_ctx* ctx, const double* w, int64_t N, int64_t ld, unsigned char** w8_out, bool* integral_out,
                           double* wsum_out);

int gd_dtype_bytes(int dtype);
int gd_check_device_array(gd_ctx* ctx, const char* what, const void* base, int64_t rows, int64_t cols, int64_t rs, int64_t cs, int sz);
int gd_wait_for_stream(gd_ctx* ctx, void* producer);

int gd_fail(gd_ctx* ctx, int code, const char* fmt, ...);
void gd_comm_release(gd_ctx* ctx);
bool gd_ctx_alive(gd_ctx* ctx);
int gd_stream_priority(gd_ctx* ctx, int level);
void* gd_scratch(gd_ctx* ctx, int64_t bytes);
void* gd_scratch2(gd_ctx* ctx, int64_t bytes);

#define GD_HIP(call)                                                                                 \
    do {                                                                                             \
        hipError_t e__ = (call);                                                                     \
        if (e__ != hipSuccess)                                                                       \
            return gd_fail(ctx, e__ == hipErrorOutOfMemory ? GD_ERR_NOMEM : GD_ERR_HIP, "%s: %s (%s:%d)", #call, \
                           hipGetErrorString(e__), __FILE__, __LINE__);                              \
    } while (0)

#define GD_KERNEL_CHECK() GD_HIP(hipGetLastError())

#define GD_TRY(call)              \
    do {                          \
        const int rc__ = (call);  \
        if (rc__) return rc__;    \
    } while (0)

#define GD_REQUIRE(cond, msg)                                   \
    do {                                                        \
        if (!(cond)) return gd_fail(ctx, GD_ERR_BADARG, "%s", msg); \
    } while (0)

#define GD_REQUIRE_ROWS(lo, hi) GD_REQUIRE(ctx->cols && (lo) >= 0 && (hi) <= ctx->N && (lo) < (hi), "bad row range")
#define GD_REQUIRE_COLUMNS_BELOW(cols, count, bound)                                                                  \
    do {                                                                                                              \
        for (int64_t i__ = 0; i__ < (int64_t)(count); ++i__) GD_REQUIRE((cols)[i__] >= 0 && (cols)[i__] < (bound), "column index out of range"); \
    } while (0)
#define GD_REQUIRE_COLUMNS(cols, count) GD_REQUIRE_COLUMNS_BELOW(cols, count, ctx->n + GD_EXTRA_COLS)
#define GD_REQUIRE_SAMPLE_COLUMNS(cols, count) GD_REQUIRE_COLUMNS_BELOW(cols, count, ctx->n)

template <class F>
inline auto gd_by_flag(bool flag, F&& f) {
    if (flag) return f(std::true_type{});
    return f(std::false_type{});
}

#define WAVE 64

typedef double gd_f64x2 __attribute__((ext_vector_type(2)));
typedef unsigned int gd_u32x4 __attribute__((ext_vector_type(4)));
__device__ __forceinline__ double2 gload_d2(const double* p) {
    const gd_f64x2 v = *(const __attribute__((address_space(1))) gd_f64x2*)p;
    return make_double2(v.x, v.y);
}
__device__ __forceinline__ uint4 gload_u4(const void* p) {
    const gd_u32x4 v = *(const __attribute__((address_space(1))) gd_u32x4*)p;
    return make_uint4(v.x, v.y, v.z, v.w);
}

template <class T>
__device__ __forceinline__ T wave_sum(T v) {
#pragma unroll
    for (int o = 32; o > 0; o >>= 1) v += __shfl_down(v, o, WAVE);
    return v;
}
__device__ __forceinline__ double wave_min(double v) {
#pragma unroll
    for (int o = 32; o > 0; o >>= 1) v = fmin(v, __shfl_down(v, o, WAVE));
    return v;
}
__device__ __forceinline__ double wave_max(double v) {
#pragma unroll
    for (int o = 32; o > 0; o >>= 1) v = fmax(v, __shfl_down(v, o, WAVE));
    return v;
}

template <class T>
__device__ __forceinline__ T block_sum(T v, T* red) {
    v = wave_sum(v);
    const int lane = threadIdx.x & 63, wv = threadIdx.x >> 6, nw = (blockDim.x + 63) >> 6;
    __syncthreads();
    if (lane == 0) red[wv] = v;
    __syncthreads();
    T r = 0;
    if (threadIdx.x == 0)
        for (int i = 0; i < nw; ++i) r += red[i];
    return r;
// ... 24 lines not shown
```

getdist_amd/csrc/stats.hip:

```cpp
#include "ctx.hpp"

#include <algorithm>
#include <cmath>

#define NBLK_STREAM 1024

template <bool HAS_W, class F>
__device__ __forceinline__ void stream_xw(const double* __restrict__ x, const double* __restrict__ w, int64_t lo,
                                          int64_t hi, F f) {
    const int64_t gtid = (int64_t)blockIdx.x * blockDim.x + threadIdx.x;
    const int64_t gsz = (int64_t)gridDim.x * blockDim.x;
    const int64_t a = (lo + 1) & ~(int64_t)1, b = hi & ~(int64_t)1;
    if (b <= a) {
        if (gtid == 0)
            for (int64_t i = lo; i < hi; ++i) f(x[i], HAS_W ? w[i] : 1.0);
        return;
    }
    if (gtid == 0) {
        if (lo < a) f(x[lo], HAS_W ? w[lo] : 1.0);
        if (b < hi) f(x[b], HAS_W ? w[b] : 1.0);
    }
    for (int64_t i = a + 2 * gtid; i < b; i += 2 * gsz) {
        const double2 xv = *reinterpret_cast<const double2*>(x + i);
        double2 wv = make_double2(1.0, 1.0);
// ... 2062 lines not shown
        GD_KERNEL_CHECK();
        return GD_OK;
    };
    const int P = (hi - lo) <= 15000000 ? 3 : 4;
    int rc;
    for (int pass = 0; pass < P; ++pass)
        if ((rc = radix_pass(pass))) return rc;
    GD_HIP(hipMemsetAsync(d_cnt, 0, (size_t)ncols * QK_MAX * 4 + 256, ctx->stream));
    {
        dim3 grid(nblk, ncols);
        gd_by_flag(ctx->w != nullptr, [&](auto HW) {
            k_qsel_collect<HW.value><<<grid, 512, 0, ctx->stream>>>(ctx->cols, ctx->ld, d_idx, ctx->w, lo, hi, P, d_st, d_lk, d_lw, d_cnt);
        });
        GD_KERNEL_CHECK();
    }
    k_qsel_finish<<<dim3(ncols, QK_MAX), 1024, 0, ctx->stream>>>(d_st, d_lk, d_lw, d_cnt, k, P, d_out, d_cnt + (int64_t)ncols * QK_MAX,
                                                                 ctx->w || getenv("GDHIP_QSEL_WALK") ? 0 : 1);
    GD_KERNEL_CHECK();
    int overflow = 0;
    GD_TRY(gd_fetch(ctx, &overflow, d_cnt + (int64_t)ncols * QK_MAX, 4));
    GD_TRY(gd_fetch(ctx, out, d_out, (size_t)ncols * k * 8));
    GD_TRY(gd_stream_sync(ctx));
    if (!overflow) return GD_OK;
    for (int pass = P; pass < 8; ++pass)
        if ((rc = radix_pass(pass))) return rc;
    k_qsel_out<<<(ncols * k + 255) / 256, 256, 0, ctx->stream>>>(d_st, ncols, k, d_out);
    GD_KERNEL_CHECK();
    GD_TRY(gd_fetch(ctx, out, d_out, (size_t)ncols * k * 8));
    GD_TRY(gd_stream_sync(ctx));
    return GD_OK;
}

int gd_autocov_lags_batch(gd_ctx* ctx, const int32_t* cols, int32_t ncols, const double* means, int64_t k0,
                          int32_t nlags, double* out) {
    GD_REQUIRE(ctx, "null context");
    return gd_autocov_lags_range_batch(ctx, cols, ncols, means, 0, ctx->N, k0, nlags, out);
}

int gd_autocov_lags_range_batch(gd_ctx* ctx, const int32_t* cols, int32_t ncols, const double* means, int64_t row_lo,
                                int64_t row_hi, int64_t k0, int32_t nlags, double* out) {
    GD_REQUIRE(ctx && cols && means && out && nlags > 0 && ncols > 0, "bad argument");
    GD_REQUIRE(ctx->cols && k0 >= 0, "bad lag / no samples");
    GD_REQUIRE_ROWS(row_lo, row_hi);
    const int64_t NR = row_hi - row_lo;
    GD_REQUIRE_COLUMNS(cols, ncols);
    int nblk = (8 * ctx->cu_count + ncols - 1) / ncols;
    if (nblk < 16) nblk = 16;
    if (nblk > 2 * ctx->cu_count) nblk = 2 * ctx->cu_count;
    ScratchPlan sp;
    auto part = sp.take<double>((int64_t)ncols * nblk * AL);
    auto d_out = sp.take<double>((int64_t)ncols * AL);
    auto d_idx = sp.take<int32_t>(ncols);
    auto d_mean = sp.take<double>(ncols);
    GD_TRY(sp.get(ctx));
    GD_TRY(gd_h2d(ctx, d_idx, cols, (size_t)ncols * 4));
    GD_TRY(gd_h2d(ctx, d_mean, means, (size_t)ncols * 8));
    std::vector<double> h((size_t)ncols * AL);
    for (int32_t done = 0; done < nlags;) {
        const dim3 grid(nblk, ncols);
        const int NL = (nlags - done <= 8) ? 8 : AL;
        gd_by_flag(ctx->w != nullptr, [&](auto HW) {
            if (NL == 8)
                k_autocov<HW.value, 8><<<grid, 256, 0, ctx->stream>>>(ctx->cols, ctx->ld, d_idx, ctx->w, row_lo, NR, d_mean, k0 + done, part);
            else
                k_autocov<HW.value, AL><<<grid, 256, 0, ctx->stream>>>(ctx->cols, ctx->ld, d_idx, ctx->w, row_lo, NR, d_mean, k0 + done, part);
        });
        GD_KERNEL_CHECK();
        k_sum_partials_batched<<<dim3(NL, ncols), 256, 0, ctx->stream>>>(part, nblk, NL, d_out);
        GD_KERNEL_CHECK();
        GD_TRY(gd_fetch(ctx, h.data(), d_out, (size_t)ncols * NL * 8));
        GD_TRY(gd_stream_sync(ctx));
        const int take_n = (nlags - done < NL) ? nlags - done : NL;
        for (int c = 0; c < ncols; ++c)
            for (int l = 0; l < take_n; ++l) out[(size_t)c * nlags + done + l] = h[(size_t)c * NL + l];
        done += take_n;
    }
    return GD_OK;
}

int gd_autocov_lags(gd_ctx* ctx, int32_t col, double mean, int64_t k0, int32_t nlags, double* out) {
    return gd_autocov_lags_batch(ctx, &col, 1, &mean, k0, nlags, out);
}

int gd_kde_lag_sums_batch(gd_ctx* ctx, const int32_t* cols, int32_t ncols, const double* inv4s2, const int64_t* lags,
                          int32_t nlags, double* out) {
    GD_REQUIRE(ctx && cols && inv4s2 && lags && out && nlags > 0 && nlags <= 64 && ncols > 0, "bad argument");
    GD_REQUIRE(ctx->cols, "no samples uploaded");
    GD_REQUIRE_COLUMNS(cols, ncols);
    for (int i = 0; i < nlags; ++i) GD_REQUIRE(lags[i] > 0 && lags[i] < ctx->N, "lag out of range");
    const bool multi = nlags <= KDE_LAG_MAX && getenv("GDHIP_KDE_LAG_SINGLE") == nullptr;
    int per_cu = 8;
    if (const char* e = getenv("GDHIP_KDE_LAG_BLOCKS_PER_CU")) per_cu = atoi(e) > 0 ? atoi(e) : per_cu;
    int nblk = multi ? (per_cu * ctx->cu_count + ncols - 1) / ncols : (8 * ctx->cu_count + ncols * nlags - 1) / (ncols * nlags);
    if (nblk < 8) nblk = 8;
    if (nblk > 2 * ctx->cu_count) nblk = 2 * ctx->cu_count;
    ScratchPlan sp;
    auto part = sp.take<double>((int64_t)ncols * (multi ? KDE_LAG_MAX : nlags) * nblk);
    auto d_lags = sp.take<int64_t>(nlags);
    auto d_idx = sp.take<int32_t>(ncols);
    auto d_c = sp.take<double>(ncols);
    GD_TRY(sp.get(ctx));
    int order[KDE_LAG_MAX];
    int nf = 0, nn = 0;
    bool folded = false;
    if (multi && ctx->N >= 4096 && getenv("GDHIP_KDE_LAG_UNFOLDED") == nullptr) {
        int64_t K0 = ctx->N, nmax = 0;
        for (int i = 0; i < nlags; ++i)
            if (4 * lags[i] >= ctx->N) {
                order[nf++] = i;
                K0 = lags[i] < K0 ? lags[i] : K0;
            }
        for (int i = 0; i < nlags; ++i)
            if (4 * lags[i] < ctx->N) {
                order[nf + nn++] = i;
                nmax = lags[i] > nmax ? lags[i] : nmax;
            }
        folded = nf == 5 && (nn == 1 || nn == 2) && 2 * K0 <= ctx->N && nmax < 256;
    }
    if (folded) {
        int64_t sorted[KDE_LAG_MAX];
        for (int i = 0; i < nlags; ++i) sorted[i] = lags[order[i]];
        GD_TRY(gd_h2d(ctx, d_lags, sorted, (size_t)nlags * 8));
    } else {
        for (int i = 0; i < nlags && i < KDE_LAG_MAX; ++i) order[i] = i;
        GD_TRY(gd_h2d(ctx, d_lags, lags, (size_t)nlags * 8));
    }
    GD_TRY(gd_h2d(ctx, d_idx, cols, (size_t)ncols * 4));
    GD_TRY(gd_h2d(ctx, d_c, inv4s2, (size_t)ncols * 8));
    if (multi) {
        const dim3 grid(nblk, ncols);
        if (folded) {
            gd_by_flag(ctx->w != nullptr, [&](auto HW) {
                gd_by_flag(nn == 1, [&](auto ONE) {
                    k_kde_lag_folded<HW.value, 5, ONE.value ? 1 : 2><<<grid, 256, 0, ctx->stream>>>(ctx->cols, ctx->ld, d_idx, ctx->w, ctx->N, d_c,
                                                                                                    d_lags, part);
                });
            });
        } else
            gd_by_flag(ctx->w != nullptr, [&](auto HW) {
#define KDE_LAUNCH(NLV) \
    case NLV: k_kde_lag_multi<HW.value, NLV><<<grid, 256, 0, ctx->stream>>>(ctx->cols, ctx->ld, d_idx, ctx->w, ctx->N, d_c, d_lags, part); break;
                switch (nlags) {
                    KDE_LAUNCH(1) KDE_LAUNCH(2) KDE_LAUNCH(3) KDE_LAUNCH(4) KDE_LAUNCH(5) KDE_LAUNCH(6) KDE_LAUNCH(7) KDE_LAUNCH(8)
                }
#undef KDE_LAUNCH
            });
        GD_KERNEL_CHECK();
        std::vector<double> h((size_t)ncols * nblk * KDE_LAG_MAX);
        GD_TRY(gd_fetch(ctx, h.data(), part, h.size() * 8));
        GD_TRY(gd_stream_sync(ctx));
        for (int c = 0; c < ncols; ++c)
            for (int l = 0; l < nlags; ++l) {
                double sum = 0;
                for (int b = 0; b < nblk; ++b) sum += h[((size_t)c * nblk + b) * KDE_LAG_MAX + l];
                out[(size_t)c * nlags + order[l]] = sum;
            }
        return GD_OK;
    }
    const dim3 grid(nblk, nlags, ncols);
    gd_by_flag(ctx->w != nullptr, [&](auto HW) {
        k_kde_lag<HW.value><<<grid, 256, 0, ctx->stream>>>(ctx->cols, ctx->ld, d_idx, ctx->w, ctx->N, d_c, d_lags, part);
    });
    GD_KERNEL_CHECK();
    std::vector<double> h((size_t)ncols * nlags * nblk);
    GD_TRY(gd_fetch(ctx, h.data(), part, h.size() * 8));
    GD_TRY(gd_stream_sync(ctx));
    for (size_t q = 0; q < (size_t)ncols * nlags; ++q) {
        double sum = 0;
        for (int b = 0; b < nblk; ++b) sum += h[q * nblk + b];
        out[q] = sum;
    }
    return GD_OK;
}

int gd_kde_lag_sums(gd_ctx* ctx, int32_t col, double inv4s2, const int64_t* lags, int32_t nlags, double* out) {
    return gd_kde_lag_sums_batch(ctx, &col, 1, &inv4s2, lags, nlags, out);
}

}
```

getdist_amd/mcsamples.py:

```python

import copy as _copy
import logging
import os
import time

import numpy as np

from ._lib import Context
from .chains import Chains, MCSamplesError
from .densities import Density1D, Density2D, DensitiesError
from .paramnames import ParamNames
from .parampriors import ParamBounds
from .types import LikeStats, MargeStats, NoLineTableFormatter, ParamLimit, ResultTable

import threading

from ._lib import GdhipError
from .chains import (ChainView, ParamConfidenceData, ParamError, WeightedSampleError, WeightedSamples,
                     _g2_independence_vs_markov, _g2_markov_vs_second_order, _where_rows, covToCorr)
from .paramnames import ParamInfo, _PlotParamInfo

DEFAULT_SETTINGS = dict(
    ignore_rows=0.0, min_weight_ratio=1e-30, contours=[0.68, 0.95, 0.99], credible_interval_threshold=0.05,
    range_ND_contour=-1, range_confidence=0.001, corr_length_thin=0, corr_length_steps=15, converge_test_limit=0.95, fine_bins=1024, smooth_scale_1D=-1.0,
# ... 424 lines not shown
        host = [[None if o is None else to_host(o, d, np.float64).reshape(-1) for o, d in zip(per_chain(v), row)]
                for v, row in zip((weights, loglikes), descs[1:])]
        wdesc = list(descs[1])
        for k, p in enumerate(parts):
            for v in (host[0][k], host[1][k]):
                if v is not None and v.shape[0] != p.shape[0]:
                    return host_route()
        ignore_frac = 0 if int(self.ignore_rows) else self.ignore_rows
        mwr = self.min_weight_ratio

        def drop(k, count):
            parts[k] = parts[k].rows_from(count)
            host[0][k], host[1][k] = (None if v is None else v[count:] for v in (host[0][k], host[1][k]))
            if wdesc[k] is not None:
                wdesc[k] = wdesc[k].rows_from(count)

        for k in range(len(parts)):
            if ignore_lines:
                drop(k, ignore_lines)
            w = host[0][k]
            if w is not None and mwr is not None and mwr >= 0 and w.size and np.min(w) < np.max(w) * mwr:
                return host_route()
            if ignore_frac:
                drop(k, int(ignore_frac) if ignore_frac >= 1 else int(round(parts[k].shape[0] * ignore_frac)))
        numrows = sum(p.shape[0] for p in parts)
        if numrows == 0:
            return host_route()
        fixed = []
        first = parts[0]
        if first.shape[0]:
            ends = [ctx.fetch_device_array(first.row(i)) for i in (0, -1)]
            if ends[0] is None:
                return host_route()
            fixed = self._fixed_columns(np.vstack(ends), lambda i: ctx.fetch_device_array(first.column(i)).reshape(-1))
        gone = {i for i, _ in fixed}
        keep = [i for i in range(first.shape[1]) if i not in gone]
        if not keep:
            return host_route()
        wparts = temp = None
        if weights is not None:
            wparts, temp = [], []
            for k, w in enumerate(host[0]):
                if wdesc[k] is None:
                    buf = ctx.alloc(max(w.nbytes, 8))
                    buf.from_host(np.ascontiguousarray(w))
                    temp.append(buf)
                    wdesc[k] = devarray.DevArray(buf.ptr, w.shape, (1,), devarray.GD_DT_F64, None, None, buf)
                wparts.append(wdesc[k])
            if len({d.dtype for d in wparts}) != 1:
                for k, w in enumerate(host[0]):
                    if wparts[k].dtype != devarray.GD_DT_F64:
                        buf = ctx.alloc(max(w.nbytes, 8))
                        buf.from_host(np.ascontiguousarray(w))
                        temp.append(buf)
                        wparts[k] = devarray.DevArray(buf.ptr, w.shape, (1,), devarray.GD_DT_F64, None, None, buf)
        try:
            if not ctx.upload_device(parts, wparts, keep if fixed else None):
                return host_route()
        finally:
            for buf in temp or ():
                buf.free()
        if is_list:
            self.chain_offsets = np.cumsum(np.array([0] + [p.shape[0] for p in parts]))
        self._device_installed = True
        stack = (lambda vs: None if vs[0] is None else np.ascontiguousarray(np.concatenate(vs), dtype=np.float64))
        return dict(numrows=numrows, n=len(keep), weights=stack(host[0]), loglikes=stack(host[1]), fixed=fixed)

    def _second_lane(self):
        own = ("ctx", "_idx_cols", "density1D", "timings", "_helper_exec", "_lane_exec", "_twin", "_lane")
        if self._twin is None:
            import copy

            twin = copy.copy(self)
            twin.ctx = self._context_factory(self._device)
            twin.ctx.attach(self.ctx)
            twin._idx_cols, twin.density1D, twin.timings = {}, {}, {}
            twin._helper_exec = twin._lane_exec = twin._twin = None
            twin._lane = 1
            self._twin = twin
        self._nlanes = 2
        self._twin.__dict__.update({k: v for k, v in list(self.__dict__.items()) if k not in own})
        return self._twin

    def _lane_thread(self, twin):
        if self._lane_exec is None:
            from concurrent.futures import ThreadPoolExecutor

            self._lane_exec = ThreadPoolExecutor(max_workers=1, thread_name_prefix="gdhip-lane",
                                                 initializer=twin.ctx.bind_thread)
        return self._lane_exec

    def _finish_pending(self):
        pend, self._pending_results = getattr(self, "_pending_results", None), None
        if pend is not None:
            pend.wait()
        if getattr(self.ctx, "h", None) is not None and hasattr(self.ctx, "batch2d_finish"):
            self.ctx.batch2d_finish()
        twin = getattr(self, "_twin", None)
        if twin is not None and getattr(twin, "_pending_results", None) is not None:
            pend, twin._pending_results = twin._pending_results, None
            pend.wait()

    def _drop_second_lane(self):
        self._finish_pending()
        if getattr(self, "_lane_exec", None) is not None:
            self._lane_exec.shutdown(wait=True)
        self._lane_exec = None
        if self._twin is not None:
            if self._twin._helper_exec is not None:
                self._twin._helper_exec.shutdown(wait=True)
            self._twin.ctx.close()
            self._twin = None
        self._nlanes = 1

    def _sample_set_changing(self):
        self._drop_second_lane()
        self._chain_stats_cache = {}
        self._loglikes_col = None
        self.indep_thin = 0
        self._idx_cols = {}
        self.mean_loglike = None
        self._like_mode = None

    def _upload(self, filter_weights=True):
        self._sample_set_changing()
        self.__dict__["_mirror_assigned"] = False
        w = self.weights
        if self._device_installed:
            self._device_installed = False
            return
        if (filter_weights and self.chain_offsets is None and w is not None and self.min_weight_ratio is not None
                and self.min_weight_ratio >= 0):
            mx, mn = np.max(w), np.min(w)
            if mn < mx * self.min_weight_ratio:
                thr = mx * self.min_weight_ratio
                keep = w > thr
                on_device = self._device_edit_applies() and np.any(keep)
                if on_device:
                    self.ctx.upload(self.samples, w)
                    on_device = self._select_on_device(rows=("weight_gt", thr))
                if not on_device:
                    self.samples = self.samples[keep]
                self.weights = w = w[keep]
                if self.loglikes is not None:
                    self.loglikes = self.loglikes[keep]
                self.numrows = len(w)
                if on_device:
                    return
        share = getattr(self, "_column_share", None)
        if share is not None:
            share.upload(self.ctx, self.samples, w)
        else:
            self.ctx.upload(self.samples, w)

    def parName(self, i, starDerived=False):
        par = self.paramNames.names[i]
        return par.name + "*" if starDerived and par.isDerived else par.name

    def parLabel(self, i):
        if isinstance(i, str):
            return self.paramNames.parWithName(i).label
        return self.paramNames.names[i].label

    def getUpper(self, name):
        par = self.paramNames.parWithName(name)
        return getattr(par, "limmax", None) if par else None
# ... 332 lines not shown
                    logging.warning("Computing two tail limits")
                continue
            if k.startswith("max_frac_twotail") and k[len("max_frac_twotail"):].isdigit():
                self._max_frac_overrides = dict(getattr(self, "_max_frac_overrides", {}))
                self._max_frac_overrides[int(k[len("max_frac_twotail"):]) - 1] = float(v)
                continue
            if k == "no_warning_params":
                self.no_warning_params = v.split() if isinstance(v, str) else list(v)
                continue
            if k == "no_warning_chi2_params":
                self.no_warning_chi2_params = v in (True, "T", "t", "True", "true", 1)
                continue
            if k not in DEFAULT_SETTINGS:
                raise SettingError("unknown setting: %s" % k)
            cur = DEFAULT_SETTINGS[k]
            if isinstance(cur, bool):
                v = v in (True, "T", "t", "True", "true", 1)
            elif isinstance(cur, int) and not isinstance(v, bool):
                v = int(v)
            elif isinstance(cur, float):
                v = float(v)
            setattr(self, k, v)
        if doUpdate:
            self.needs_update = True

    def setRanges(self, ranges):
        if isinstance(ranges, dict):
            for nm, rng in ranges.items():
                self.ranges.setRange(nm, rng)
        else:
            for nm, rng in zip(self.paramNames.list(), ranges):
                self.ranges.setRange(nm, rng)
        self.needs_update = True

    def _after_base_statistics(self):
        self.density1D = {}
        self._initLimits()
        for par in self.paramNames.names:
            par.N_eff_kde = None
            par._ranges_done = False
        self._nd_limits_done = False
        self._marge_done = None
        self.likeStats = None
        self.needs_update = False

    def _initLimits(self):
        for par in self.paramNames.names:
            par.limmin = self.ranges.getLower(par.name)
            par.limmax = self.ranges.getUpper(par.name)
            par.has_limits_bot = par.limmin is not None
            par.has_limits_top = par.limmax is not None
            par.periodic = par.name in self.ranges.periodic

    CONV_TWO_STREAMS_PAIRS = (64, 400)
    KOPT_FIRST_FRACTION = 0.5
    KOPT_SPLIT_MIN = 256

    def _get1DNeff(self, par, param):
        if par.N_eff_kde is None:
            par.N_eff_kde = self.getEffectiveSamplesGaussianKDE(param, scale=par.sigma_range)
        return par.N_eff_kde

    def _initParamRanges(self, j, paramConfid=None):
        self._init_params([self._col(j)])
        return self.paramNames.names[self._col(j)]

    def _setNDLimits(self):
        if self._nd_limits_done:
            return
        ctx = self.ctx
        col = getattr(self, "_loglikes_col", None)
        if col is None:
            col = ctx.set_extra_column(ctx.EXTRA_COLS - 1, self.loglikes)
        contours = np.asarray(self.contours, dtype=np.float64)
        thr = ctx.quantiles([col], (self.norm * contours)[None, :])[0]
        lims = np.empty((len(contours), self.n, 2))
        for i, (c, t) in enumerate(zip(contours, thr)):
            lims[i] = ctx.col_minmax(list(range(self.n)), cond_col=-1 if c >= 1 else col, cond_below=t)
        for j, par in enumerate(self.paramNames.names):
            par.ND_limit_bot = lims[:, j, 0].copy()
            par.ND_limit_top = lims[:, j, 1].copy()
        self._nd_limits_done = True

    def _init_params(self, js, lag_probe=False):
        todo = [j for j in dict.fromkeys(js) if not getattr(self.paramNames.names[j], "_ranges_done", False)]
        if not todo:
            return
        rc = self.range_confidence
        fracs = np.array([rc, 1 - rc] + list(np.linspace(0.1, 0.9, 9)))
        targets = np.tile(self.norm * fracs, (len(todo), 1))
        if lag_probe:
            q, lags = self.ctx.quantiles_probe(todo, targets, self._minmax_of(todo), self.means[todo])
            q = np.asarray(q)
            if lags is not None:
                self._lag_prefetch = (todo, 8, _Done(lags))
        else:
            q = np.asarray(self.ctx.quantiles(todo, targets, minmax=self._minmax_of(todo)))
        err_v = np.asarray(self.sddev)[todo]
        confids = np.empty_like(q)
        confids[:, 0] = np.asarray(self._col_min)[todo]
        confids[:, 1:-1] = q[:, 2:]
        confids[:, -1] = np.asarray(self._col_max)[todo]
        diffs = confids[:, 4:] - confids[:, :-4]
        scale_v = np.min(diffs, axis=1) / 1.049
        flat_v = (np.all(diffs > (err_v * 1.049)[:, None], axis=1) & np.all(diffs < (scale_v * 1.5)[:, None], axis=1)).tolist()
        for row, j in enumerate(todo):
            par = self.paramNames.names[j]
            par.err = self.sddev[j]
            par.mean = self.means[j]
            par.param_min = self._col_min[j]
            par.param_max = self._col_max[j]
            par.range_min, par.range_max = q[row, 0], q[row, 1]
            scale = scale_v[row]
            if flat_v[row]:
                par.sigma_range = scale
            else:
                par.sigma_range = min(par.err, scale)
            if self.range_ND_contour >= 0 and self.loglikes is not None:
                self._setNDLimits()
                if self.range_ND_contour >= par.ND_limit_bot.size:
                    raise SettingError("range_ND_contour should be -1 (off), or an index into the computed contour levels")
                par.range_min = min(max(par.range_min - par.err, par.ND_limit_bot[self.range_ND_contour]), par.range_min)
                par.range_max = max(max(par.range_max + par.err, par.ND_limit_top[self.range_ND_contour]), par.range_max)
            smooth_1D = par.sigma_range * 0.4
            if par.has_limits_bot:
                if par.range_min - par.limmin > 2 * smooth_1D and par.param_min - par.limmin > smooth_1D:
                    par.has_limits_bot = False
                else:
                    par.range_min = par.limmin
            if par.has_limits_top:
                if par.limmax - par.range_max > 2 * smooth_1D and par.limmax - par.param_max > smooth_1D:
                    par.has_limits_top = False
                else:
                    par.range_max = par.limmax
            if not par.has_limits_bot:
                par.range_min -= smooth_1D * 2
            if not par.has_limits_top:
                par.range_max += smooth_1D * 2
            par.has_limits = par.has_limits_top or par.has_limits_bot
            par._ranges_done = True

    def prepareParams(self, params=None, neff=True):
        if self.needs_update:
            self.updateBaseStatistics()
        js = list(range(self.n)) if params is None else [self._col(p) for p in params]
        todo = [j for j in js if self.paramNames.names[j].N_eff_kde is None]
        fused = (bool(todo) and self.sampler not in ("nested", "uncorrelated") and self.numrows // 10 + 1 >= 8
                 and hasattr(self.ctx, "quantiles_probe") and os.environ.get("GETDIST_AMD_FUSED_PROBE", "1") == "1"
                 and all(not getattr(self.paramNames.names[j], "_ranges_done", False) for j in todo))
        if fused:
            with _Phase(self, "prep.ranges"):
                self._init_params(js, lag_probe=True)
        elif (todo and self._lane == 0 and not self._timing and self.sampler not in ("nested", "uncorrelated")
                and len(todo) >= 2 and os.environ.get("GETDIST_AMD_OVERLAP_NEFF", "1") == "1"):
            twin = self._second_lane()
            self._nlanes = 1
            nl = min(8, self.numrows // 10 + 1)
            self._lag_prefetch = (todo, nl, self._lane_thread(twin).submit(
                twin.ctx.autocov_lags_batch, todo, self.means[todo], 0, nl))
        with _Phase(self, "prep.ranges"), _FastThreadSwitch(getattr(self, "_lag_prefetch", None) is not None):
            self._init_params(js)
        _hostlog("prep: ranges done")
        if neff:
            with _Phase(self, "prep.neff"):
                self._neff_batch(js)
            _hostlog("prep: N_eff done")
        return js

    def _bin_edge_arrays(self, js, borderfrac=0.1):
        names = self.paramNames.names
        n = max(js) + 1
        rmin, rmax, pmin, pmax = np.zeros(n), np.zeros(n), np.zeros(n), np.zeros(n)
        lim_b, lim_t = np.zeros(n, dtype=bool), np.zeros(n, dtype=bool)
        for j in js:
            p = names[j]
            rmin[j], rmax[j], pmin[j], pmax[j] = p.range_min, p.range_max, p.param_min, p.param_max
            lim_b[j], lim_t[j] = bool(p.has_limits_bot), bool(p.has_limits_top)
        border = (rmax - rmin) * borderfrac
        binmin = np.minimum(pmin, rmin)
        binmin = np.where(lim_b, binmin, binmin - border)
        binmax = np.maximum(pmax, rmax)
        binmax = np.where(lim_t, binmax, binmax + border)
        return binmin, binmax

    @staticmethod
    def _bin_edges(par, num_fine_bins, borderfrac=0.1):
        border = (par.range_max - par.range_min) * borderfrac
        binmin = min(par.param_min, par.range_min)
        if not par.has_limits_bot:
            binmin -= border
        binmax = max(par.param_max, par.range_max)
        if not par.has_limits_top:
            binmax += border
        fine_width = (binmax - binmin) / (num_fine_bins - 1)
        return fine_width, binmin, binmax

    def getAutoBandwidth1D(self, bins, par, param, mult_bias_correction_order=None, kernel_order=1, N_eff=None):
        if N_eff is None:
            N_eff = self._get1DNeff(par, param)
        h, status = self.ctx.isj1d(np.asarray(bins, dtype=np.float64)[None, :], [N_eff])
        return self._bandwidth_1d(None if status[0] else h[0], par, N_eff, mult_bias_correction_order, kernel_order)

    def _no_bandwidth_warning(self, par):
        return par.name in self.no_warning_params or (
            bool(self.no_warning_chi2_params) and ("chi2_" in par.name or "minuslog" in par.name))

    def _bandwidth_1d(self, h, par, N_eff, mult_bias_correction_order, kernel_order):
        if h is None:
            logging.warning("1D auto bandwidth failed. Using fallback: zero f in _bandwidth_fixed_point (non-convergence)")
        bin_range = max(par.param_max, par.range_max) - min(par.param_min, par.range_min)
        if h is None or h < 0.01 * N_eff ** (-1.0 / 5) * (par.range_max - par.range_min) / bin_range:
            hnew = 1.06 * par.sigma_range * N_eff ** (-1.0 / 5) / bin_range
            if not self._no_bandwidth_warning(par):
                msg = f"auto bandwidth for {par.name} very small or failed (h={h},N_eff={N_eff}). Using fallback (h={hnew})"
                if self.raise_on_bandwidth_errors:
                    raise BandwidthError(msg)
                logging.warning(msg)
            h = hnew
        par.kde_h = h
        m = self.mult_bias_correction_order if mult_bias_correction_order is None else mult_bias_correction_order
        if kernel_order > 1:
            m = max(m, 1)
        if m:
            return h * N_eff ** (1.0 / 5 - 1.0 / (4 * m + 5))
        return h

    def get1DDensity(self, name, **kwargs):
        if self.needs_update:
            self.updateBaseStatistics()
        if not kwargs:
            j, par = self._parAndNumber(name)
            if par is not None and par.name in self.density1D:
                return self.density1D[par.name]
        return self.get1DDensityGridData(name, **kwargs)

# ... 901 lines not shown
```

include/gdhip.h:

```cpp
#ifndef GDHIP_H
#define GDHIP_H

#include <stdint.h>

#ifdef __cplusplus
extern "C" {
#endif

typedef struct gd_ctx gd_ctx;

typedef enum gd_status {
    GD_OK = 0,
    GD_ERR_BADARG = -1,
    GD_ERR_NOMEM = -2,
    GD_ERR_HIP = -3,
    GD_ERR_EMPTY = -4,
    GD_ERR_SOLVER = -5,
    GD_ERR_FFT = -6,
    GD_ERR_NODEVICE = -7,
    GD_ERR_TIMEOUT = -8
} gd_status;

int gd_device_count(void);
int gd_create(int device, gd_ctx** out);
// ... 303 lines not shown
#define GD_TAB_SPLINE2 36
#define GD_TAB_MAX_TABLES 4
#define GD_TAB_MAX_DOUBLES 4194304
typedef struct gd_expr_table {
    int32_t kind;
    int32_t deriv;
    int32_t nx, ny;
    const double* p0;
    const double* p1;
    const double* p2;
    double left, right;
} gd_expr_table;
int gd_expr_eval_tab(gd_ctx* ctx, const int32_t* code, int32_t ncode, const double* consts, int32_t nconst, int32_t dst,
                     int32_t dst_arg, int64_t lo, int64_t hi, void* host_out, double* stats_out, const gd_expr_table* tables,
                     int32_t ntab);

int gd_circ_convolve(gd_ctx* ctx, int32_t n0, int32_t n1, const double* a, const double* b, double* out);
int gd_convolve1d_direct(gd_ctx* ctx, const double* x, int64_t nx, const double* y, int64_t ny, double* out_full);
int gd_autoconvolve(gd_ctx* ctx, int32_t col, double mean, int32_t use_weights, const double* x_host, int64_t nx, int64_t s,
                    int64_t n, int32_t normalize, double* out);

int gd_like_stats(gd_ctx* ctx, int32_t col, double* out8);


#define GD_BATCH2D_META 32
#define GD_BATCH2D_NEED_NEFF (-20)

typedef struct gd_param2d {
    double range_min, range_max;
    double param_min, param_max;
    double sigma_range, err;
    double mean, var;
    double neff;
    int32_t has_limits_bot, has_limits_top, periodic;
    int32_t owned;
} gd_param2d;

typedef struct gd_batch2d_settings {
    int32_t fine_bins_2D, boundary_correction_order, mult_bias_correction_order, num_bins_2D;
    double smooth_scale_2D, max_corr_2D;
    double norm, sum_w2;
    int32_t uncorrelated_sampler;
    int32_t raise_on_bandwidth_errors;
    int32_t want_levels, ncontours;
    const double* contours;
    int32_t two_streams_min;
    int32_t two_streams_split;
    int32_t kopt_split_min;
    double kopt_first_fraction;
    int32_t first_batch, max_batch;
    double max_batch_bytes;
    int32_t comm_exchange;
    int32_t bandwidths_only;
    const double* pair_neff;
    const double* bandwidths;
    int32_t results_in_flight;
} gd_batch2d_settings;

typedef int (*gd_neff_exchange_fn)(void* user, double* neff_n, int32_t n);

int gd_batch2d_grid_sizes(const gd_batch2d_settings* settings, int32_t n, const double* corr, const int32_t* pairs,
                          int32_t P, int32_t* F_out);
int gd_density2d_batch(gd_ctx* ctx, gd_ctx* twin, const gd_batch2d_settings* settings, gd_param2d* params, int32_t n,
                       const double* corr, const double* cov, const double* lag_probe, const int32_t* pairs, int32_t P,
                       gd_neff_exchange_fn exchange, void* exchange_user, void* grids_pinned, int64_t grids_doubles,
                       int32_t* status_pinned, double* meta, double* levels, int32_t* level_status, int32_t* tokens_out2);
#define GD_BATCH1D_META 9

typedef struct gd_density1d_settings {
    int32_t fine_bins, num_bins, boundary_correction_order, mult_bias_correction_order;
    double smooth_scale_1D;
    double norm, sum_w2;
    int32_t uncorrelated_sampler;
    int32_t raise_on_bandwidth_errors;
} gd_density1d_settings;

int gd_density1d_batch(gd_ctx* ctx, const gd_density1d_settings* settings, gd_param2d* params, int32_t n, const int32_t* cols,
                       int32_t B, double* P_out, double* hist_out, double* meta);

int gd_batch2d_finish(gd_ctx* ctx);
int gd_batch2d_invalidate(gd_ctx* ctx);
int gd_batch2d_exchanges(gd_ctx* ctx, int64_t* count_out);


int gd_comm_rccl_path(char* buf, int32_t len, int32_t* preloaded_out);
int gd_upload_shard(gd_ctx* ctx, const double* X_cols, int64_t N, int64_t n, int64_t col_first, int64_t col_count,
                    int64_t col_stride, const double* weights);
int gd_comm_share_columns(gd_ctx* ctx, const int64_t* first_by_rank );
int gd_comm_unique_id(void* id128_out);
int gd_comm_init(gd_ctx* ctx, int32_t world, int32_t rank, const void* id128);
int gd_comm_info(gd_ctx* ctx, int32_t* world_out, int32_t* rank_out);
int gd_comm_abandon(gd_ctx* ctx);
int gd_comm_destroy(gd_ctx* ctx);
int gd_comm_allgather(gd_ctx* ctx, const double* send, int64_t count, double* recv);
int gd_comm_allreduce_sum(gd_ctx* ctx, double* inout, int64_t count);
int gd_comm_allgather_dev(gd_ctx* ctx, const void* d_send, int64_t count, void* d_recv);
int gd_comm_allreduce_sum_dev(gd_ctx* ctx, const void* d_send, int64_t count, void* d_recv);

#ifdef __cplusplus
}
#endif
#endif
```

Baseline: 49710.

## Prepare params natively and enqueue N_eff lag sums and prebinning ahead

Adds a native gd_prepare_params entry point that computes parameter ranges in C. It also speculatively enqueues two jobs: the KDE lag-sum N_eff work on the main stream, and the 8-bit prebinning of 2D columns on a twin context's stream. Later batch calls check whether the speculated work matches their request, consume the result if it does and discard it otherwise. The aim is to hide prep latency and Python round trips behind GPU work, at the cost of substantial bookkeeping, global owner maps and possible wasted work.

```diff
diff --git a/getdist_amd/_lib.py b/getdist_amd/_lib.py
--- a/getdist_amd/_lib.py
+++ b/getdist_amd/_lib.py
@@ -141,6 +141,8 @@
     "gd_batch2d_finish": (C.c_int, [_p]),
     "gd_batch2d_invalidate": (C.c_int, [_p]),
     "gd_batch2d_exchanges": (C.c_int, [_p, C.POINTER(C.c_int64)]),
+    "gd_prepare_params": (C.c_int, [_p, _p, _p, _pi32, _i32, _pd, _pd, _pd, _pd, _pd, _pd, _pd, _pd, C.POINTER(C.c_int32), _p]),
+    "gd_prepare_ahead_counts": (C.c_int, [_p, C.POINTER(C.c_int64)]),
     "gd_comm_rccl_path": (C.c_int, [C.c_char_p, C.c_int32, C.POINTER(C.c_int32)]),
     "gd_upload_shard": (C.c_int, [_p, _p, _i64, _i64, _i64, _i64, _i64, _p]),
     "gd_comm_share_columns": (C.c_int, [_p, C.POINTER(C.c_int64)]),
@@ -266,6 +268,16 @@
             fn.argtypes = args
         _lib = lib
     return _lib
+
+
+class PrepareSettings(C.Structure):
+
+    _fields_ = [("fine_bins_2D", C.c_int32), ("auto_bandwidth", C.c_int32), ("uncorrelated_sampler", C.c_int32),
+                ("ahead", C.c_int32)]
+
+
+PREPARED_PARAM = np.dtype([("range_min", np.float64), ("range_max", np.float64), ("sigma_range", np.float64),
+                           ("has_limits_bot", np.int32), ("has_limits_top", np.int32)])
 
 
 def _dp(a):
@@ -828,6 +840,29 @@
                                                    _dp(out), _dp(means), _dp(probe), C.byref(done)))
         return out, (probe if done.value else None)
 
+    def prepare_params(self, cols, targets, minmax, means, variances, err, limits, has_bot, has_top, twin=None, fine_bins_2D=0,
+                       auto_bandwidth=False, uncorrelated_sampler=False, ahead=0):
+        cols = _i32arr(cols)
+        m = len(cols)
+        targets = _f64arr(targets).reshape(m, 11)
+        mm = _f64arr(minmax).reshape(m, 2)
+        means, variances, err = _f64arr(means), _f64arr(variances), _f64arr(err)
+        limits = _f64arr(limits).reshape(m, 2)
+        out, probe = np.zeros_like(targets), np.zeros((m, 8))
+        recs = np.zeros(m, dtype=PREPARED_PARAM)
+        recs["has_limits_bot"], recs["has_limits_top"] = has_bot, has_top
+        settings = PrepareSettings(int(fine_bins_2D), int(bool(auto_bandwidth)), int(bool(uncorrelated_sampler)), int(ahead))
+        done = C.c_int32(0)
+        self._check(self.lib.gd_prepare_params(self.h, None if twin is None else twin.h, C.byref(settings), _ip(cols), m, _dp(targets),
+                                               _dp(mm), _dp(means), _dp(variances), _dp(err), _dp(limits), _dp(out), _dp(probe),
+                                               C.byref(done), recs.ctypes.data))
+        return out, (probe if done.value else None), recs
+
+    def prepare_ahead_counts(self):
+        out = np.zeros(3, dtype=np.int64)
+        self._check(self.lib.gd_prepare_ahead_counts(self.h, out.ctypes.data_as(_pi64)))
+        return tuple(int(v) for v in out)
+
     def autocov_lags(self, col, mean, k0, nlags):
         out = np.zeros(nlags)
         self._check(self.lib.gd_autocov_lags(self.h, int(col), float(mean), int(k0), int(nlags), _dp(out)))
diff --git a/getdist_amd/csrc/batch2d.hip b/getdist_amd/csrc/batch2d.hip
--- a/getdist_amd/csrc/batch2d.hip
+++ b/getdist_amd/csrc/batch2d.hip
@@ -5,6 +5,143 @@
 namespace {
 
 gd_ctx* C(void* h) { return (gd_ctx*)h; }
+
+struct Ahead {
+    std::mutex mu_neff, mu_prebin;
+    struct {
+        bool pending = false;
+        std::vector<int32_t> cols;
+        std::vector<double> inv4s2;
+        std::vector<int64_t> lags;
+        int64_t N = 0;
+        const double *samples = nullptr, *weights = nullptr;
+        gd_kde_lag_ticket t{};
+    } neff;
+    struct {
+        bool pending = false;
+        std::vector<int32_t> cols;
+        std::vector<void*> bufs;
+    } prebin;
+    hipEvent_t ev_neff = nullptr, ev_prebin = nullptr;
+    void* d_block = nullptr;
+    int64_t d_bytes = 0;
+    double* pinned = nullptr;
+    int64_t pinned_bytes = 0;
+    unsigned long long* bad_pinned = nullptr;
+    int64_t bad_words = 0;
+    std::atomic<int64_t> enqueued{0}, consumed{0}, discarded{0};
+};
+
+std::mutex g_prebin_mu;
+std::map<const void*, gd_ctx*> g_prebin_owner;
+
+Ahead* ahead_if(gd_ctx* ctx) {
+    return ctx && ctx->batch_state ? (Ahead*)((gdb::State*)ctx->batch_state)->ahead : nullptr;
+}
+
+void settle_neff(gd_ctx* ctx, Ahead& A, bool used) {
+    if (!A.neff.pending) return;
+    (void)hipEventSynchronize(A.ev_neff);
+    A.neff.pending = false;
+    ((gdb::State*)ctx->batch_state)->neff_ahead.store(false);
+    ++(used ? A.consumed : A.discarded);
+}
+std::vector<const void*> settle_prebin(gd_ctx* owner, Ahead& A, bool used, const std::vector<const void*>& rebinned = {}) {
+    std::vector<const void*> bad;
+    if (!A.prebin.pending) return bad;
+    const bool ran = hipEventSynchronize(A.ev_prebin) == hipSuccess;
+    gdb::State& st = *(gdb::State*)owner->batch_state;
+    const int m = (int)A.prebin.cols.size();
+    for (int c = 0; c < m; ++c) {
+        const void* buf = A.prebin.bufs[c];
+        if (ran && A.bad_pinned[A.bad_pinned[m + c]] == 0) continue;
+        bad.push_back(buf);
+        if (std::find(rebinned.begin(), rebinned.end(), buf) != rebinned.end()) continue;
+        std::lock_guard<std::mutex> gs(st.mu);
+        auto it = st.idx.find(std::make_tuple((int)A.prebin.cols[c], 256, 1));
+        if (it != st.idx.end() && it->second.ptr == buf) it->second.valid = false;
+    }
+    A.prebin.pending = false;
+    {
+        std::lock_guard<std::mutex> g(g_prebin_mu);
+        for (const void* buf : A.prebin.bufs) g_prebin_owner.erase(buf);
+    }
+    ++((used && bad.empty()) ? A.consumed : A.discarded);
+    return bad;
+}
+void drop_ahead(gd_ctx* ctx) {
+    Ahead* A = ahead_if(ctx);
+    if (!A) return;
+    {
+        std::lock_guard<std::mutex> g(A->mu_neff);
+        settle_neff(ctx, *A, false);
+    }
+    std::lock_guard<std::mutex> g(A->mu_prebin);
+    (void)settle_prebin(ctx, *A, false);
+}
+
+bool take_neff_ahead(gd_ctx* ctx, const int32_t* cols, int32_t ncols, const double* inv4s2, const int64_t* lags, int32_t nlags,
+                     double* out) {
+    Ahead* A = ahead_if(ctx);
+    if (!A) return false;
+    std::lock_guard<std::mutex> g(A->mu_neff);
+    if (!A->neff.pending) return false;
+    const auto& p = A->neff;
+    bool same = p.N == ctx->N && p.samples == ctx->cols && p.weights == ctx->w && ctx->w_sel == 0 && cols && inv4s2 && lags &&
+                (int32_t)p.cols.size() == ncols && (int32_t)p.lags.size() == nlags &&
+                memcmp(p.lags.data(), lags, (size_t)nlags * 8) == 0;
+    std::vector<int> row_of(same ? ncols : 0, -1);
+    for (int c = 0; c < ncols && same; ++c) {
+        for (int q = 0; q < ncols && row_of[c] < 0; ++q)
+            if (p.cols[q] == cols[c] && memcmp(&p.inv4s2[q], &inv4s2[c], 8) == 0) row_of[c] = q;
+        same = row_of[c] >= 0;
+        for (int b = 0; b < c && same; ++b) same = cols[b] != cols[c];
+    }
+    const bool ran = hipEventSynchronize(A->ev_neff) == hipSuccess;
+    settle_neff(ctx, *A, same && ran);
+    if (!(same && ran)) return false;
+    std::vector<double> sums((size_t)ncols * nlags);
+    gd_kde_lag_sums_reduce(&p.t, A->pinned, sums.data());
+    for (int c = 0; c < ncols; ++c) memcpy(out + (size_t)c * nlags, &sums[(size_t)row_of[c] * nlags], (size_t)nlags * 8);
+    return true;
+}
+
+int meet_prebin_ahead(gd_ctx* on, int32_t ncols, void* const* d_idx, int32_t B, const void* const* ix, const void* const* iy) {
+    gd_ctx* owner = nullptr;
+    {
+        std::lock_guard<std::mutex> g(g_prebin_mu);
+        if (g_prebin_owner.empty()) return 0;
+        auto look = [&](const void* p) {
+            if (owner) return;
+            auto it = g_prebin_owner.find(p);
+            if (it != g_prebin_owner.end()) owner = it->second;
+        };
+        for (int q = 0; q < ncols && !owner; ++q) look(d_idx[q]);
+        for (int q = 0; q < B && !owner; ++q) {
+            if (ix) look(ix[q]);
+            if (iy) look(iy[q]);
+        }
+    }
+    Ahead* A = owner && gd_ctx_alive(owner) ? ahead_if(owner) : nullptr;
+    if (!A) return 0;
+    std::lock_guard<std::mutex> g(A->mu_prebin);
+    if (!A->prebin.pending) return 0;
+    std::vector<const void*> rebinned, fresh;
+    for (const void* buf : A->prebin.bufs) {
+        bool again = false, read = false;
+        for (int q = 0; q < ncols && !again; ++q) again = d_idx[q] == buf;
+        for (int q = 0; q < B && !read; ++q) read = (ix && ix[q] == buf) || (iy && iy[q] == buf);
+        if (again)
+            rebinned.push_back(buf);
+        else if (read)
+            fresh.push_back(buf);
+    }
+    const std::vector<const void*> bad = settle_prebin(owner, *A, !fresh.empty(), rebinned);
+    for (const void* buf : fresh)
+        if (std::find(bad.begin(), bad.end(), buf) != bad.end())
+            return gd_fail(on, GD_ERR_SOLVER, "samples outside the byte-index grid: use the u16 path");
+    return 0;
+}
 
 const gdb::Ops kOps = {
      [](void* h) { return gd_bind_thread(C(h)); },
@@ -17,12 +154,19 @@
      [](void* h, int64_t bytes, void** out) { return gd_dev_alloc(C(h), bytes, out); },
      [](void* h, void* p) { return gd_dev_free(C(h), p); },
     [](void* h, const int32_t* cols, int32_t ncols, const double* binmin, const double* width, int32_t F, void* const* d_idx,
-       int64_t* bad) { return gd_prebin8_batch(C(h), cols, ncols, binmin, width, F, d_idx, bad); },
+       int64_t* bad) {
+        (void)meet_prebin_ahead(C(h), ncols, d_idx, 0, nullptr, nullptr);
+        return gd_prebin8_batch(C(h), cols, ncols, binmin, width, F, d_idx, bad);
+    },
     [](void* h, int32_t B, const void* const* ix, const void* const* iy, void* d_hist) {
+        const int rc = meet_prebin_ahead(C(h), 0, nullptr, B, ix, iy);
+        if (rc) return rc;
         return gd_hist2d_prebinned8(C(h), B, ix, iy, d_hist);
     },
     [](void* h, const int32_t* cols, int32_t ncols, const double* binmin, const double* width, void* const* d_idx, int64_t* bad,
        int32_t B, const void* const* ix, const void* const* iy, void* d_hist) {
+        const int rc = meet_prebin_ahead(C(h), ncols, d_idx, B, ix, iy);
+        if (rc) return rc;
         return gd_prebin8_hist2d(C(h), cols, ncols, binmin, width, d_idx, bad, B, ix, iy, d_hist);
     },
     [](void* h, int32_t col, double binmin, double width, int32_t F, void* d_idx) {
@@ -62,6 +206,7 @@
         return gd_autocov_lags_batch(C(h), cols, ncols, means, k0, nlags, out);
     },
     [](void* h, const int32_t* cols, int32_t ncols, const double* inv4s2, const int64_t* lags, int32_t nlags, double* out) {
+        if (take_neff_ahead(C(h), cols, ncols, inv4s2, lags, nlags, out)) return 0;
         return gd_kde_lag_sums_batch(C(h), cols, ncols, inv4s2, lags, nlags, out);
     },
     [](void* h, int32_t col, double inv4s2, const int64_t* lags, int32_t nlags, double* out) {
@@ -119,8 +264,18 @@
 void release_state(gd_ctx* ctx, bool destroy) {
     gdb::State* st = (gdb::State*)ctx->batch_state;
     if (!st) return;
+    drop_ahead(ctx);
     gdb::release_all(*st, kOps, ctx);
     if (destroy) {
+        if (Ahead* A = (Ahead*)st->ahead) {
+            if (A->ev_neff) (void)hipEventDestroy(A->ev_neff);
+            if (A->ev_prebin) (void)hipEventDestroy(A->ev_prebin);
+            if (A->d_block) (void)hipFree(A->d_block);
+            if (A->pinned) (void)hipHostFree(A->pinned);
+            if (A->bad_pinned) (void)hipHostFree(A->bad_pinned);
+            delete A;
+            st->ahead = nullptr;
+        }
         delete st;
         ctx->batch_state = nullptr;
     }
@@ -134,9 +289,163 @@
     return *(gdb::State*)ctx->batch_state;
 }
 
+Ahead& ahead_of(gd_ctx* ctx) {
+    gdb::State& st = state_of(ctx);
+    if (!st.ahead) st.ahead = new Ahead();
+    return *(Ahead*)st.ahead;
+}
+
+bool prepare_ahead_enabled() {
+    const char* e = getenv("GDHIP_PREPARE_AHEAD");
+    return !(e && atoi(e) == 0);
+}
+
+int enqueue_prebin_ahead(gd_ctx* ctx, gd_ctx* twin, Ahead& A, const int32_t* cols, int32_t ncols, const double* minmax,
+                         const gd_prepared_param* recs) {
+    gdb::State& st = state_of(ctx);
+    gdb::Pool pool{st, kOps, ctx};
+    std::vector<int32_t> todo;
+    std::vector<double> b0, w;
+    std::vector<void*> bufs;
+    for (int c = 0; c < ncols; ++c) {
+        gd_param2d p;
+        memset(&p, 0, sizeof p);
+        p.range_min = recs[c].range_min, p.range_max = recs[c].range_max, p.param_min = minmax[2 * c], p.param_max = minmax[2 * c + 1];
+        p.has_limits_bot = recs[c].has_limits_bot, p.has_limits_top = recs[c].has_limits_top;
+        double lo, hi;
+        gdb::bin_edges(p, &lo, &hi);
+        const double fw = (hi - lo) / 255;
+        if (!(fw > 0) || !std::isfinite(fw) || !std::isfinite(lo)) continue;
+        gdb::IdxCol col;
+        {
+            std::lock_guard<std::mutex> g(st.mu);
+            col = st.idx[std::make_tuple((int)cols[c], 256, 1)];
+        }
+        if (col.valid && col.binmin == lo && col.width == fw) continue;
+        if (!col.ptr) {
+            int rc = 0;
+            col.ptr = pool.take(ctx->N + 64, &rc);
+            if (!col.ptr) return rc;
+            std::lock_guard<std::mutex> g(st.mu);
+            gdb::IdxCol& e = st.idx[std::make_tuple((int)cols[c], 256, 1)];
+            e.ptr = col.ptr, e.valid = false;
+        }
+        todo.push_back(cols[c]), b0.push_back(lo), w.push_back(fw), bufs.push_back(col.ptr);
+    }
+    const int m = (int)todo.size();
+    if (!m) return 0;
+    if (A.bad_words < 2 * (int64_t)m) {
+        if (A.bad_pinned) (void)hipHostFree(A.bad_pinned);
+        A.bad_pinned = nullptr, A.bad_words = 0;
+        if (hipHostMalloc((void**)&A.bad_pinned, (size_t)(2 * m + 64) * 8, hipHostMallocDefault) != hipSuccess) return GD_ERR_NOMEM;
+        A.bad_words = 2 * m + 64;
+    }
+    memset(A.bad_pinned, 0xff, (size_t)m * 8);
+    if (!A.ev_prebin && hipEventCreateWithFlags(&A.ev_prebin, hipEventDisableTiming) != hipSuccess) return GD_ERR_HIP;
+    int rc = gd_prebin8_enqueue(twin, todo.data(), m, b0.data(), w.data(), bufs.data(), A.bad_pinned);
+    const bool recorded = hipEventRecord(A.ev_prebin, twin->stream) == hipSuccess;
+    if (rc || !recorded) {
+        (void)hipStreamSynchronize(twin->stream);
+        return rc ? rc : GD_ERR_HIP;
+    }
+    {
+        std::lock_guard<std::mutex> g(st.mu);
+        for (int q = 0; q < m; ++q) {
+            gdb::IdxCol& e = st.idx[std::make_tuple((int)todo[q], 256, 1)];
+            e.binmin = b0[q], e.width = w[q], e.valid = true;
+        }
+    }
+    A.prebin.cols = todo, A.prebin.bufs = bufs, A.prebin.pending = true;
+    {
+        std::lock_guard<std::mutex> g(g_prebin_mu);
+        for (void* buf : bufs) g_prebin_owner[buf] = ctx;
+    }
+    ++A.enqueued;
+    return 0;
+}
+
+int enqueue_neff_ahead(gd_ctx* ctx, Ahead& A, const int32_t* cols, int32_t ncols, const double* probe, const double* vars,
+                       const double* err, const gd_prepared_param* recs) {
+    const int64_t N = ctx->N;
+    if (std::min<int64_t>(8, N / 10 + 1) != 8) return 0;
+    for (size_t q = 0; q < (size_t)ncols * 8; ++q)
+        if (std::isnan(probe[q])) return 0;
+    std::vector<double> sr(ncols);
+    for (int c = 0; c < ncols; ++c) sr[c] = recs[c].sigma_range;
+    gdb::LagPlan lp;
+    if (gdb::lag_plan(N, ncols, 8, probe, vars, sr.data(), err, gdb::kNeffMinCorr, lp) >= 0) return 0;
+    const int L = (int)lp.lags.size();
+    for (int64_t k : lp.lags)
+        if (!(k > 0 && k < N)) return 0;
+    const int64_t partials = gd_kde_lag_sums_partials(ctx, ncols, L);
+    if (partials <= 0) return 0;
+    const int64_t dev_bytes = partials * 8 + (int64_t)ncols * 16 + 4096, host_bytes = partials * 8;
+    if (A.d_bytes < dev_bytes) {
+        if (A.d_block) (void)hipFree(A.d_block);
+        A.d_block = nullptr, A.d_bytes = 0;
+        if (hipMalloc(&A.d_block, (size_t)dev_bytes) != hipSuccess) return GD_ERR_NOMEM;
+        A.d_bytes = dev_bytes;
+    }
+    if (A.pinned_bytes < host_bytes) {
+        if (A.pinned) (void)hipHostFree(A.pinned);
+        A.pinned = nullptr, A.pinned_bytes = 0;
+        if (hipHostMalloc((void**)&A.pinned, (size_t)host_bytes, hipHostMallocDefault) != hipSuccess) return GD_ERR_NOMEM;
+        A.pinned_bytes = host_bytes;
+    }
+    if (!A.ev_neff && hipEventCreateWithFlags(&A.ev_neff, hipEventDisableTiming) != hipSuccess) return GD_ERR_HIP;
+    const int rc = gd_kde_lag_sums_enqueue(ctx, cols, ncols, lp.inv4s2.data(), lp.lags.data(), L, A.d_block, A.pinned, &A.neff.t);
+    const bool recorded = hipEventRecord(A.ev_neff, ctx->stream) == hipSuccess;
+    if (rc || !recorded) {
+        (void)hipStreamSynchronize(ctx->stream);
+        return rc ? rc : GD_ERR_HIP;
+    }
+    A.neff.cols.assign(cols, cols + ncols), A.neff.inv4s2 = lp.inv4s2, A.neff.lags = lp.lags;
+    A.neff.N = N, A.neff.samples = ctx->cols, A.neff.weights = ctx->w, A.neff.pending = true;
+    state_of(ctx).neff_ahead.store(true);
+    ++A.enqueued;
+    return 0;
+}
+
 }
 
 extern "C" {
+
+int gd_prepare_params(gd_ctx* ctx, gd_ctx* twin, const gd_prepare_settings* settings, const int32_t* cols, int32_t ncols,
+                      const double* targets, const double* minmax, const double* means, const double* vars, const double* err,
+                      const double* limits, double* quantiles_out, double* probe_out, int32_t* probe_done,
+                      gd_prepared_param* recs) {
+    GD_REQUIRE(ctx && settings && cols && targets && minmax && means && vars && err && limits && quantiles_out && probe_out &&
+                   probe_done && recs && ncols > 0,
+               "bad argument");
+    GD_REQUIRE(ctx->cols, "no samples uploaded");
+    GD_REQUIRE_SAMPLE_COLUMNS(cols, ncols);
+    GD_HIP(hipSetDevice(ctx->device));
+    drop_ahead(ctx);
+    GD_TRY(gd_quantiles_mm_probe(ctx, cols, ncols, 0, ctx->N, targets, 11, minmax, quantiles_out, means, probe_out, probe_done));
+    for (int c = 0; c < ncols; ++c)
+        gdb::prepare_tail(quantiles_out + (size_t)11 * c, minmax[2 * c], minmax[2 * c + 1], err[c], limits[2 * c], limits[2 * c + 1], &recs[c]);
+    if (!settings->ahead || !prepare_ahead_enabled() || ctx->w_sel != 0) return GD_OK;
+    try {
+        Ahead& A = ahead_of(ctx);
+        std::lock_guard<std::mutex> g1(A.mu_neff), g2(A.mu_prebin);
+        int rc = 0;
+        if ((settings->ahead & 2) && twin && twin != ctx && twin->cols == ctx->cols && !ctx->w && settings->fine_bins_2D == 256 &&
+            (int64_t)ncols * (ncols - 1) / 2 >= gdb::kByteIndexMinPairs)
+            rc = enqueue_prebin_ahead(ctx, twin, A, cols, ncols, minmax, recs);
+        if (!rc && (settings->ahead & 1) && settings->auto_bandwidth && !settings->uncorrelated_sampler && *probe_done)
+            rc = enqueue_neff_ahead(ctx, A, cols, ncols, probe_out, vars, err, recs);
+        if (rc) (void)hipGetLastError();
+    } catch (const std::exception&) {
+    }
+    return GD_OK;
+}
+
+int gd_prepare_ahead_counts(gd_ctx* ctx, int64_t* out3) {
+    GD_REQUIRE(ctx && out3, "null argument");
+    out3[0] = out3[1] = out3[2] = 0;
+    if (Ahead* A = ahead_if(ctx)) out3[0] = A->enqueued.load(), out3[1] = A->consumed.load(), out3[2] = A->discarded.load();
+    return GD_OK;
+}
 
 int gd_batch2d_grid_sizes(const gd_batch2d_settings* settings, int32_t n, const double* corr, const int32_t* pairs, int32_t P,
                           int32_t* F_out) {
@@ -169,6 +478,7 @@
     } catch (const std::exception& e) {
         rc = gd_fail(ctx, GD_ERR_NOMEM, "gd_density2d_batch: %s", e.what());
     }
+    drop_ahead(ctx);
     return rc;
 }
 
diff --git a/getdist_amd/csrc/batch2d.hpp b/getdist_amd/csrc/batch2d.hpp
--- a/getdist_amd/csrc/batch2d.hpp
+++ b/getdist_amd/csrc/batch2d.hpp
@@ -153,6 +153,43 @@
     *binmin = lo, *binmax = hi;
 }
 
+static inline void prepare_tail(const double q[11], double col_min, double col_max, double err, double limmin, double limmax,
+                                gd_prepared_param* rec) {
+    double confids[11];
+    confids[0] = col_min;
+    for (int k = 0; k < 9; ++k) confids[1 + k] = q[2 + k];
+    confids[10] = col_max;
+    double diffs[7];
+    for (int k = 0; k < 7; ++k) diffs[k] = confids[k + 4] - confids[k];
+    double mn = diffs[0];
+    for (int k = 1; k < 7; ++k) mn = np_minimum(mn, diffs[k]);
+    const double scale = mn / 1.049;
+    bool flat = true;
+    const double lo = err * 1.049, hi = scale * 1.5;
+    for (int k = 0; k < 7; ++k) flat = flat && (diffs[k] > lo) && (diffs[k] < hi);
+    rec->sigma_range = flat ? scale : (scale < err ? scale : err);
+    double range_min = q[0], range_max = q[1];
+    const double smooth_1D = rec->sigma_range * 0.4;
+    if (rec->has_limits_bot) {
+        if (range_min - limmin > 2 * smooth_1D && col_min - limmin > smooth_1D)
+            rec->has_limits_bot = 0;
+        else
+            range_min = limmin;
+    }
+    if (rec->has_limits_top) {
+        if (limmax - range_max > 2 * smooth_1D && limmax - col_max > smooth_1D)
+            rec->has_limits_top = 0;
+        else
+            range_max = limmax;
+    }
+    if (!rec->has_limits_bot) range_min -= smooth_1D * 2;
+    if (!rec->has_limits_top) range_max += smooth_1D * 2;
+    rec->range_min = range_min, rec->range_max = range_max;
+}
+
+static constexpr int kByteIndexMinPairs = 64;
+static constexpr double kNeffMinCorr = 0.05;
+
 struct NeffInput {
     int64_t N;
     double norm, sum_w2;
@@ -214,6 +251,48 @@
     if (rc) return rc;
     *neff_out = py_pow(in.norm, 2.0) / Nn;
     return 0;
+}
+
+struct LagPlan {
+    std::vector<double> inv4s2;
+    std::vector<int64_t> maxoffs, lags;
+    int ntail = 0;
+};
+static inline int lag_plan(int64_t N, int m, int nl, const double* lag0, const double* var, const double* sigma_range,
+                           const double* err, double min_corr, LagPlan& lp) {
+    const int64_t max_off = N / 10;
+    lp.inv4s2.assign(m, NAN), lp.maxoffs.assign(m, 0), lp.lags.clear(), lp.ntail = 0;
+    bool all_uncorrelated_at_lag_1 = true;
+    for (int row = 0; row < m; ++row) {
+        double c[8];
+        for (int k = 0; k < nl; ++k) c[k] = lag0[(size_t)row * nl + k] / (double)(N - k) / var[row];
+        int first_below = -1;
+        for (int k = 0; k < nl; ++k)
+            if (!(c[k] > min_corr * c[0])) {
+                first_below = k;
+                break;
+            }
+        if (first_below != 1) all_uncorrelated_at_lag_1 = false;
+        double corrlen;
+        if (first_below >= 0) {
+            double sum = 0.0;
+            for (int k = 1; k < first_below; ++k) sum += c[k];
+            corrlen = c[0] + 2 * sum;
+        } else if (nl == max_off + 1) {
+            corrlen = c[0];
+        } else {
+            return row;
+        }
+        const double sr = sigma_range[row];
+        const double kstd = ((isnan(sr) || sr == 0.0) ? err[row] : sr) * 0.2;
+        lp.inv4s2[row] = 1.0 / (4 * py_pow(kstd, 2.0));
+        lp.maxoffs[row] = (int64_t)(corrlen * 1.5) + 4;
+    }
+    const int64_t uncorr_len = N / 2;
+    for (int64_t k = uncorr_len; k < uncorr_len + 5; ++k) lp.lags.push_back(k);
+    for (int64_t k : {1, 2})
+        if (k <= N / 10 && (k == 1 || !all_uncorrelated_at_lag_1)) lp.lags.push_back(k), ++lp.ntail;
+    return -1;
 }
 
 struct Plan {
@@ -295,6 +374,8 @@
     Pending prev;
     void* aux = nullptr;
     void* aux2 = nullptr;
+    void* ahead = nullptr;
+    std::atomic<bool> neff_ahead{false};
     int64_t exchanges_entered = 0;
     static constexpr int64_t kCacheLimit = 16LL << 30;
 };
@@ -566,7 +647,7 @@
 
     double* M(int k) { return meta + (size_t)k * GD_BATCH2D_META; }
 
-    int neff_batch(const std::vector<int>& js, bool owned_only, double min_corr = 0.05) {
+    int neff_batch(const std::vector<int>& js, bool owned_only, double min_corr = kNeffMinCorr) {
         std::vector<int32_t> todo;
         for (int j : js)
             if (isnan(par[j].neff) && (!owned_only || (par[j].owned & 1))) todo.push_back(j);
@@ -592,48 +673,28 @@
             for (int row = 0; row < m; ++row) means[row] = par[todo[row]].mean;
             GDB_DEV(h, ops.autocov_lags_batch(h, todo.data(), m, means.data(), 0, nl, lag0.data()));
         }
-        std::vector<double> kstd(m), inv4s2(m);
-        std::vector<int64_t> maxoffs(m);
-        bool all_uncorrelated_at_lag_1 = true;
-        for (int row = 0; row < m; ++row) {
-            const gd_param2d& p = par[todo[row]];
-            double c[8];
-            for (int k = 0; k < nl; ++k) c[k] = lag0[(size_t)row * nl + k] / (double)(N - k) / p.var;
-            int first_below = -1;
-            for (int k = 0; k < nl; ++k)
-                if (!(c[k] > min_corr * c[0])) {
-                    first_below = k;
-                    break;
-                }
-            if (first_below != 1) all_uncorrelated_at_lag_1 = false;
-            double corrlen;
-            if (first_below >= 0) {
-                double sum = 0.0;
-                for (int k = 1; k < first_below; ++k) sum += c[k];
-                corrlen = c[0] + 2 * sum;
-            } else if (nl == max_off + 1) {
-                corrlen = c[0];
-            } else {
+        LagPlan lp;
+        {
+            std::vector<double> var(m), sr(m), er(m);
+            for (int row = 0; row < m; ++row) {
+                const gd_param2d& p = par[todo[row]];
+                var[row] = p.var, sr[row] = p.sigma_range, er[row] = p.err;
+            }
+            const int long_row = lag_plan(N, m, nl, lag0.data(), var.data(), sr.data(), er.data(), min_corr, lp);
+            if (long_row >= 0) {
                 char buf[160];
                 snprintf(buf, sizeof buf, "column %d: the chain's correlation outlasts the 8-lag probe (getCorrelationLength's long route)",
-                         (int)todo[row]);
+                         (int)todo[long_row]);
                 return fail(GD_BATCH2D_NEED_NEFF, buf);
             }
-            const double sr = p.sigma_range;
-            kstd[row] = ((isnan(sr) || sr == 0.0) ? p.err : sr) * 0.2;
-            inv4s2[row] = 1.0 / (4 * py_pow(kstd[row], 2.0));
-            maxoffs[row] = (int64_t)(corrlen * 1.5) + 4;
-        }
-        std::vector<int64_t> lags;
-        const int64_t uncorr_len = N / 2;
-        for (int64_t k = uncorr_len; k < uncorr_len + 5; ++k) lags.push_back(k);
-        int ntail = 0;
-        for (int64_t k : {1, 2})
-            if (k <= N / 10 && (k == 1 || !all_uncorrelated_at_lag_1)) lags.push_back(k), ++ntail;
+        }
+        const std::vector<double>& inv4s2 = lp.inv4s2;
+        const std::vector<int64_t>&maxoffs = lp.maxoffs, &lags = lp.lags;
+        const int ntail = lp.ntail;
         const int L = (int)lags.size();
         std::vector<double> sums((size_t)m * L);
         mark("neff: probe done");
-        if (hold_neff_for_binning) {
+        if (hold_neff_for_binning && !st.neff_ahead.load()) {
             const auto t0 = std::chrono::steady_clock::now();
             while (!bin_launching.load() && std::chrono::steady_clock::now() - t0 < std::chrono::milliseconds(2)) std::this_thread::yield();
             int hold_us = 120;
@@ -753,7 +814,7 @@
             const std::vector<int>& members = classes.at(F);
             const int B = (int)members.size();
             int rc = 0;
-            if (F == 256 && (unit_weights || byte_index_weights) && B >= 64) {
+            if (F == 256 && (unit_weights || byte_index_weights) && B >= kByteIndexMinPairs) {
                 std::vector<int> cols;
                 std::vector<char> seen(n, 0);
                 for (int k : members)
diff --git a/getdist_amd/csrc/binning.hip b/getdist_amd/csrc/binning.hip
--- a/getdist_amd/csrc/binning.hip
+++ b/getdist_amd/csrc/binning.hip
@@ -1354,15 +1354,18 @@
     return rc;
 }
 
-int gd_prebin8_batch(gd_ctx* ctx, const int32_t* cols, int32_t ncols, const double* binmin, const double* width, int32_t F,
-                     void* const* d_idx_out, int64_t* bad_out) {
-    GD_REQUIRE(ctx && cols && binmin && width && d_idx_out && bad_out && ncols > 0, "bad argument");
-    GD_REQUIRE(ctx->cols, "no samples uploaded");
-    GD_REQUIRE(F >= 2 && F <= 256, "byte indices need fine_bins_2D <= 256");
-    for (int c = 0; c < ncols; ++c) GD_REQUIRE(cols[c] >= 0 && cols[c] < ctx->n + GD_EXTRA_COLS && d_idx_out[c], "bad column");
-    const BucketRoute R = bucket_route(ctx, cols, ncols, binmin, width, d_idx_out);
+struct Prebin8Launch {
+    BucketRoute R;
+    std::vector<int> fp_of;
+    int nfp = 0;
+    unsigned long long *d_bad = nullptr, *d_bad_bq = nullptr;
+};
+static int prebin8_launch(gd_ctx* ctx, const int32_t* cols, int32_t ncols, const double* binmin, const double* width, int32_t F,
+                          void* const* d_idx_out, Prebin8Launch& PL) {
+    PL.R = bucket_route(ctx, cols, ncols, binmin, width, d_idx_out);
+    const BucketRoute& R = PL.R;
     std::vector<PrebinCol8> hc;
-    std::vector<int> fp_of((size_t)ncols, -1);
+    PL.fp_of.assign((size_t)ncols, -1);
     for (int c = 0; c < ncols; ++c) {
         if (R.slot_of[c] >= 0) continue;
         PrebinCol8 r;
@@ -1370,10 +1373,10 @@
         r.idx = (unsigned char*)d_idx_out[c];
         r.binmin = binmin[c];
         r.width = width[c];
-        fp_of[c] = (int)hc.size();
+        PL.fp_of[c] = (int)hc.size();
         hc.push_back(r);
     }
-    const int nfp = (int)hc.size();
+    const int nfp = PL.nfp = (int)hc.size();
     BucketRouteLayout L(ctx, R);
     ScratchPlan sp;
     auto d_c = sp.take<PrebinCol8>(nfp);
@@ -1389,14 +1392,40 @@
         if (nblk < 1) nblk = 1;
         k_prebin8_batch<<<dim3(nblk, nfp), 256, 0, ctx->stream>>>(d_c, ctx->N, F, d_bad);
         GD_KERNEL_CHECK();
-    }
-    unsigned long long* d_bad_bq = nullptr;
-    if (!R.recs.empty()) GD_TRY(bucket_route_launch<true>(ctx, R, L, F, &d_bad_bq));
-    std::vector<unsigned long long> hb((size_t)nfp), hq(R.recs.size());
-    if (nfp) GD_TRY(gd_fetch(ctx, hb.data(), d_bad, (size_t)nfp * 8));
-    if (!R.recs.empty()) GD_TRY(gd_fetch(ctx, hq.data(), d_bad_bq, hq.size() * 8));
+        PL.d_bad = d_bad;
+    }
+    if (!R.recs.empty()) GD_TRY(bucket_route_launch<true>(ctx, R, L, F, &PL.d_bad_bq));
+    return GD_OK;
+}
+
+int gd_prebin8_batch(gd_ctx* ctx, const int32_t* cols, int32_t ncols, const double* binmin, const double* width, int32_t F,
+                     void* const* d_idx_out, int64_t* bad_out) {
+    GD_REQUIRE(ctx && cols && binmin && width && d_idx_out && bad_out && ncols > 0, "bad argument");
+    GD_REQUIRE(ctx->cols, "no samples uploaded");
+    GD_REQUIRE(F >= 2 && F <= 256, "byte indices need fine_bins_2D <= 256");
+    for (int c = 0; c < ncols; ++c) GD_REQUIRE(cols[c] >= 0 && cols[c] < ctx->n + GD_EXTRA_COLS && d_idx_out[c], "bad column");
+    Prebin8Launch PL;
+    GD_TRY(prebin8_launch(ctx, cols, ncols, binmin, width, F, d_idx_out, PL));
+    const int nfp = PL.nfp;
+    std::vector<unsigned long long> hb((size_t)nfp), hq(PL.R.recs.size());
+    if (nfp) GD_TRY(gd_fetch(ctx, hb.data(), PL.d_bad, (size_t)nfp * 8));
+    if (!PL.R.recs.empty()) GD_TRY(gd_fetch(ctx, hq.data(), PL.d_bad_bq, hq.size() * 8));
     GD_TRY(gd_stream_sync(ctx));
-    for (int c = 0; c < ncols; ++c) bad_out[c] = (int64_t)(R.slot_of[c] >= 0 ? hq[R.slot_of[c]] : hb[fp_of[c]]);
+    for (int c = 0; c < ncols; ++c) bad_out[c] = (int64_t)(PL.R.slot_of[c] >= 0 ? hq[PL.R.slot_of[c]] : hb[PL.fp_of[c]]);
+    return GD_OK;
+}
+
+int gd_prebin8_enqueue(gd_ctx* ctx, const int32_t* cols, int32_t ncols, const double* binmin, const double* width,
+                       void* const* d_idx_out, unsigned long long* bad_pinned) {
+    GD_REQUIRE(ctx && cols && binmin && width && d_idx_out && bad_pinned && ncols > 0, "bad argument");
+    GD_REQUIRE(ctx->cols && !ctx->w, "index columns are enqueued ahead for unit weights only");
+    for (int c = 0; c < ncols; ++c) GD_REQUIRE(cols[c] >= 0 && cols[c] < ctx->n && d_idx_out[c], "bad column");
+    Prebin8Launch PL;
+    GD_TRY(prebin8_launch(ctx, cols, ncols, binmin, width, 256, d_idx_out, PL));
+    const int nfp = PL.nfp;
+    for (int c = 0; c < ncols; ++c) bad_pinned[ncols + c] = (unsigned long long)(PL.R.slot_of[c] >= 0 ? nfp + PL.R.slot_of[c] : PL.fp_of[c]);
+    if (nfp) GD_TRY(gd_fetch_pinned(ctx, bad_pinned, PL.d_bad, (size_t)nfp * 8));
+    if (!PL.R.recs.empty()) GD_TRY(gd_fetch_pinned(ctx, bad_pinned + nfp, PL.d_bad_bq, PL.R.recs.size() * 8));
     return GD_OK;
 }
 
diff --git a/getdist_amd/csrc/ctx.hpp b/getdist_amd/csrc/ctx.hpp
--- a/getdist_amd/csrc/ctx.hpp
+++ b/getdist_amd/csrc/ctx.hpp
@@ -121,6 +121,19 @@
 int gd_check_device_array(gd_ctx* ctx, const char* what, const void* base, int64_t rows, int64_t cols, int64_t rs, int64_t cs, int sz);
 int gd_wait_for_stream(gd_ctx* ctx, void* producer);
 
+struct gd_kde_lag_ticket {
+    int32_t ncols, nlags, nblk;
+    int order[8];
+};
+extern "C" {
+int64_t gd_kde_lag_sums_partials(const gd_ctx* ctx, int32_t ncols, int32_t nlags);
+int gd_kde_lag_sums_enqueue(gd_ctx* ctx, const int32_t* cols, int32_t ncols, const double* inv4s2, const int64_t* lags,
+                            int32_t nlags, void* d_block, double* pinned, gd_kde_lag_ticket* t);
+void gd_kde_lag_sums_reduce(const gd_kde_lag_ticket* t, const double* h, double* out);
+int gd_prebin8_enqueue(gd_ctx* ctx, const int32_t* cols, int32_t ncols, const double* binmin, const double* width,
+                       void* const* d_idx_out, unsigned long long* bad_pinned);
+}
+
 int gd_fail(gd_ctx* ctx, int code, const char* fmt, ...);
 void gd_comm_release(gd_ctx* ctx);
 bool gd_ctx_alive(gd_ctx* ctx);
diff --git a/getdist_amd/csrc/stats.hip b/getdist_amd/csrc/stats.hip
--- a/getdist_amd/csrc/stats.hip
+++ b/getdist_amd/csrc/stats.hip
@@ -2168,28 +2168,20 @@
     return gd_autocov_lags_batch(ctx, &col, 1, &mean, k0, nlags, out);
 }
 
-int gd_kde_lag_sums_batch(gd_ctx* ctx, const int32_t* cols, int32_t ncols, const double* inv4s2, const int64_t* lags,
-                          int32_t nlags, double* out) {
-    GD_REQUIRE(ctx && cols && inv4s2 && lags && out && nlags > 0 && nlags <= 64 && ncols > 0, "bad argument");
-    GD_REQUIRE(ctx->cols, "no samples uploaded");
-    GD_REQUIRE_COLUMNS(cols, ncols);
-    for (int i = 0; i < nlags; ++i) GD_REQUIRE(lags[i] > 0 && lags[i] < ctx->N, "lag out of range");
-    const bool multi = nlags <= KDE_LAG_MAX && getenv("GDHIP_KDE_LAG_SINGLE") == nullptr;
+static int kde_lag_blocks(const gd_ctx* ctx, int32_t ncols, int32_t nlags, bool multi) {
     int per_cu = 8;
     if (const char* e = getenv("GDHIP_KDE_LAG_BLOCKS_PER_CU")) per_cu = atoi(e) > 0 ? atoi(e) : per_cu;
     int nblk = multi ? (per_cu * ctx->cu_count + ncols - 1) / ncols : (8 * ctx->cu_count + ncols * nlags - 1) / (ncols * nlags);
     if (nblk < 8) nblk = 8;
     if (nblk > 2 * ctx->cu_count) nblk = 2 * ctx->cu_count;
-    ScratchPlan sp;
-    auto part = sp.take<double>((int64_t)ncols * (multi ? KDE_LAG_MAX : nlags) * nblk);
-    auto d_lags = sp.take<int64_t>(nlags);
-    auto d_idx = sp.take<int32_t>(ncols);
-    auto d_c = sp.take<double>(ncols);
-    GD_TRY(sp.get(ctx));
-    int order[KDE_LAG_MAX];
+    return nblk;
+}
+
+static int kde_lag_multi_launch(gd_ctx* ctx, const int32_t* cols, int32_t ncols, const double* inv4s2, const int64_t* lags,
+                                int32_t nlags, int nblk, double* part, int64_t* d_lags, int32_t* d_idx, double* d_c, int* order) {
     int nf = 0, nn = 0;
     bool folded = false;
-    if (multi && ctx->N >= 4096 && getenv("GDHIP_KDE_LAG_UNFOLDED") == nullptr) {
+    if (ctx->N >= 4096 && getenv("GDHIP_KDE_LAG_UNFOLDED") == nullptr) {
         int64_t K0 = ctx->N, nmax = 0;
         for (int i = 0; i < nlags; ++i)
             if (4 * lags[i] >= ctx->N) {
@@ -2213,36 +2205,89 @@
     }
     GD_TRY(gd_h2d(ctx, d_idx, cols, (size_t)ncols * 4));
     GD_TRY(gd_h2d(ctx, d_c, inv4s2, (size_t)ncols * 8));
-    if (multi) {
-        const dim3 grid(nblk, ncols);
-        if (folded) {
-            gd_by_flag(ctx->w != nullptr, [&](auto HW) {
-                gd_by_flag(nn == 1, [&](auto ONE) {
-                    k_kde_lag_folded<HW.value, 5, ONE.value ? 1 : 2><<<grid, 256, 0, ctx->stream>>>(ctx->cols, ctx->ld, d_idx, ctx->w, ctx->N, d_c,
-                                                                                                    d_lags, part);
-                });
+    const dim3 grid(nblk, ncols);
+    if (folded) {
+        gd_by_flag(ctx->w != nullptr, [&](auto HW) {
+            gd_by_flag(nn == 1, [&](auto ONE) {
+                k_kde_lag_folded<HW.value, 5, ONE.value ? 1 : 2><<<grid, 256, 0, ctx->stream>>>(ctx->cols, ctx->ld, d_idx, ctx->w, ctx->N, d_c,
+                                                                                                d_lags, part);
             });
-        } else
-            gd_by_flag(ctx->w != nullptr, [&](auto HW) {
+        });
+    } else
+        gd_by_flag(ctx->w != nullptr, [&](auto HW) {
 #define KDE_LAUNCH(NLV) \
     case NLV: k_kde_lag_multi<HW.value, NLV><<<grid, 256, 0, ctx->stream>>>(ctx->cols, ctx->ld, d_idx, ctx->w, ctx->N, d_c, d_lags, part); break;
-                switch (nlags) {
-                    KDE_LAUNCH(1) KDE_LAUNCH(2) KDE_LAUNCH(3) KDE_LAUNCH(4) KDE_LAUNCH(5) KDE_LAUNCH(6) KDE_LAUNCH(7) KDE_LAUNCH(8)
-                }
+            switch (nlags) {
+                KDE_LAUNCH(1) KDE_LAUNCH(2) KDE_LAUNCH(3) KDE_LAUNCH(4) KDE_LAUNCH(5) KDE_LAUNCH(6) KDE_LAUNCH(7) KDE_LAUNCH(8)
+            }
 #undef KDE_LAUNCH
-            });
-        GD_KERNEL_CHECK();
+        });
+    GD_KERNEL_CHECK();
+    return GD_OK;
+}
+
+void gd_kde_lag_sums_reduce(const gd_kde_lag_ticket* t, const double* h, double* out) {
+    for (int c = 0; c < t->ncols; ++c)
+        for (int l = 0; l < t->nlags; ++l) {
+            double sum = 0;
+            for (int b = 0; b < t->nblk; ++b) sum += h[((size_t)c * t->nblk + b) * KDE_LAG_MAX + l];
+            out[(size_t)c * t->nlags + t->order[l]] = sum;
+        }
+}
+
+static bool kde_lag_multi(int32_t nlags) { return nlags <= KDE_LAG_MAX && getenv("GDHIP_KDE_LAG_SINGLE") == nullptr; }
+
+int64_t gd_kde_lag_sums_partials(const gd_ctx* ctx, int32_t ncols, int32_t nlags) {
+    if (!ctx || ncols <= 0 || nlags <= 0 || !kde_lag_multi(nlags)) return 0;
+    return (int64_t)ncols * KDE_LAG_MAX * kde_lag_blocks(ctx, ncols, nlags, true);
+}
+
+int gd_kde_lag_sums_enqueue(gd_ctx* ctx, const int32_t* cols, int32_t ncols, const double* inv4s2, const int64_t* lags,
+                            int32_t nlags, void* d_block, double* pinned, gd_kde_lag_ticket* t) {
+    GD_REQUIRE(ctx && cols && inv4s2 && lags && d_block && pinned && t && nlags > 0 && ncols > 0, "bad argument");
+    GD_REQUIRE(ctx->cols, "no samples uploaded");
+    GD_REQUIRE(kde_lag_multi(nlags), "more lags than one launch takes");
+    GD_REQUIRE_SAMPLE_COLUMNS(cols, ncols);
+    for (int i = 0; i < nlags; ++i) GD_REQUIRE(lags[i] > 0 && lags[i] < ctx->N, "lag out of range");
+    const int nblk = kde_lag_blocks(ctx, ncols, nlags, true);
+    ScratchPlan sp;
+    auto part = sp.take<double>((int64_t)ncols * KDE_LAG_MAX * nblk);
+    auto d_lags = sp.take<int64_t>(nlags);
+    auto d_idx = sp.take<int32_t>(ncols);
+    auto d_c = sp.take<double>(ncols);
+    GD_TRY(sp.place(d_block));
+    t->ncols = ncols, t->nlags = nlags, t->nblk = nblk;
+    GD_TRY(kde_lag_multi_launch(ctx, cols, ncols, inv4s2, lags, nlags, nblk, part, d_lags, d_idx, d_c, t->order));
+    return gd_fetch_pinned(ctx, pinned, part, (size_t)ncols * KDE_LAG_MAX * nblk * 8);
+}
+
+int gd_kde_lag_sums_batch(gd_ctx* ctx, const int32_t* cols, int32_t ncols, const double* inv4s2, const int64_t* lags,
+                          int32_t nlags, double* out) {
+    GD_REQUIRE(ctx && cols && inv4s2 && lags && out && nlags > 0 && nlags <= 64 && ncols > 0, "bad argument");
+    GD_REQUIRE(ctx->cols, "no samples uploaded");
+    GD_REQUIRE_COLUMNS(cols, ncols);
+    for (int i = 0; i < nlags; ++i) GD_REQUIRE(lags[i] > 0 && lags[i] < ctx->N, "lag out of range");
+    const bool multi = kde_lag_multi(nlags);
+    const int nblk = kde_lag_blocks(ctx, ncols, nlags, multi);
+    ScratchPlan sp;
+    auto part = sp.take<double>((int64_t)ncols * (multi ? KDE_LAG_MAX : nlags) * nblk);
+    auto d_lags = sp.take<int64_t>(nlags);
+    auto d_idx = sp.take<int32_t>(ncols);
+    auto d_c = sp.take<double>(ncols);
+    GD_TRY(sp.get(ctx));
+    if (multi) {
+        gd_kde_lag_ticket t;
+        t.ncols = ncols, t.nlags = nlags, t.nblk = nblk;
+        GD_TRY(kde_lag_multi_launch(ctx, cols, ncols, inv4s2, lags, nlags, nblk, part, d_lags, d_idx, d_c, t.order));
         std::vector<double> h((size_t)ncols * nblk * KDE_LAG_MAX);
         GD_TRY(gd_fetch(ctx, h.data(), part, h.size() * 8));
         GD_TRY(gd_stream_sync(ctx));
-        for (int c = 0; c < ncols; ++c)
-            for (int l = 0; l < nlags; ++l) {
-                double sum = 0;
-                for (int b = 0; b < nblk; ++b) sum += h[((size_t)c * nblk + b) * KDE_LAG_MAX + l];
-                out[(size_t)c * nlags + order[l]] = sum;
-            }
+        gd_kde_lag_sums_reduce(&t, h.data(), out);
         return GD_OK;
     }
+    GD_TRY(gd_h2d(ctx, d_lags, lags, (size_t)nlags * 8));
+    GD_TRY(gd_h2d(ctx, d_idx, cols, (size_t)ncols * 4));
+    GD_TRY(gd_h2d(ctx, d_c, inv4s2, (size_t)ncols * 8));
     const dim3 grid(nblk, nlags, ncols);
     gd_by_flag(ctx->w != nullptr, [&](auto HW) {
         k_kde_lag<HW.value><<<grid, 256, 0, ctx->stream>>>(ctx->cols, ctx->ld, d_idx, ctx->w, ctx->N, d_c, d_lags, part);
diff --git a/getdist_amd/mcsamples.py b/getdist_amd/mcsamples.py
--- a/getdist_amd/mcsamples.py
+++ b/getdist_amd/mcsamples.py
@@ -530,6 +530,13 @@
         self._twin.__dict__.update({k: v for k, v in list(self.__dict__.items()) if k not in own})
         return self._twin
 
+    def _twin_context(self):
+        if self._twin is None:
+            nlanes = self._nlanes
+            self._second_lane()
+            self._nlanes = nlanes
+        return self._twin.ctx
+
     def _lane_thread(self, twin):
         if self._lane_exec is None:
             from concurrent.futures import ThreadPoolExecutor
@@ -1028,13 +1035,16 @@
             par.ND_limit_top = lims[:, j, 1].copy()
         self._nd_limits_done = True
 
-    def _init_params(self, js, lag_probe=False):
+    def _init_params(self, js, lag_probe=False, ahead=0):
         todo = [j for j in dict.fromkeys(js) if not getattr(self.paramNames.names[j], "_ranges_done", False)]
         if not todo:
             return
         rc = self.range_confidence
         fracs = np.array([rc, 1 - rc] + list(np.linspace(0.1, 0.9, 9)))
         targets = np.tile(self.norm * fracs, (len(todo), 1))
+        if (lag_probe and hasattr(self.ctx, "prepare_params") and getattr(self, "_col_min", None) is not None
+                and not (self.range_ND_contour >= 0 and self.loglikes is not None)):
+            return self._init_params_native(todo, targets, ahead)
         if lag_probe:
             q, lags = self.ctx.quantiles_probe(todo, targets, self._minmax_of(todo), self.means[todo])
             q = np.asarray(q)
@@ -1086,6 +1096,33 @@
             par.has_limits = par.has_limits_top or par.has_limits_bot
             par._ranges_done = True
 
+    def _init_params_native(self, todo, targets, ahead):
+        names = self.paramNames.names
+        pars = [names[j] for j in todo]
+        nan = np.nan
+        limits = np.array([[nan if p.limmin is None else p.limmin, nan if p.limmax is None else p.limmax] for p in pars])
+        twin = None
+        if (ahead & 2 and self._lane == 0 and self._context_factory is not None and self.weights is None
+                and len(todo) * (len(todo) - 1) // 2 >= min(64, self.CONV_TWO_STREAMS_PAIRS[0])):
+            twin = self._twin_context()
+        q, lags, recs = self.ctx.prepare_params(
+            todo, targets, self._minmax_of(todo), self.means[todo], np.asarray(self.vars)[todo], np.asarray(self.sddev)[todo],
+            limits, [bool(p.has_limits_bot) for p in pars], [bool(p.has_limits_top) for p in pars], twin=twin,
+            fine_bins_2D=self.fine_bins_2D, auto_bandwidth=self.smooth_scale_2D < 0 and not self.use_effective_samples_2D,
+            uncorrelated_sampler=self.sampler in ("nested", "uncorrelated"), ahead=ahead if twin is not None else ahead & 1)
+        if lags is not None:
+            self._lag_prefetch = (todo, 8, _Done(lags))
+        for row, (j, par) in enumerate(zip(todo, pars)):
+            par.err = self.sddev[j]
+            par.mean = self.means[j]
+            par.param_min = self._col_min[j]
+            par.param_max = self._col_max[j]
+            par.range_min, par.range_max = recs["range_min"][row], recs["range_max"][row]
+            par.sigma_range = recs["sigma_range"][row]
+            par.has_limits_bot, par.has_limits_top = bool(recs["has_limits_bot"][row]), bool(recs["has_limits_top"][row])
+            par.has_limits = par.has_limits_top or par.has_limits_bot
+            par._ranges_done = True
+
     def prepareParams(self, params=None, neff=True):
         if self.needs_update:
             self.updateBaseStatistics()
@@ -1095,8 +1132,10 @@
                  and hasattr(self.ctx, "quantiles_probe") and os.environ.get("GETDIST_AMD_FUSED_PROBE", "1") == "1"
                  and all(not getattr(self.paramNames.names[j], "_ranges_done", False) for j in todo))
         if fused:
+            ahead = 3 if (not neff and getattr(self, "_neff_share", None) is None
+                          and os.environ.get("GDHIP_PREPARE_AHEAD", "1") != "0") else 0
             with _Phase(self, "prep.ranges"):
-                self._init_params(js, lag_probe=True)
+                self._init_params(js, lag_probe=True, ahead=ahead)
         elif (todo and self._lane == 0 and not self._timing and self.sampler not in ("nested", "uncorrelated")
                 and len(todo) >= 2 and os.environ.get("GETDIST_AMD_OVERLAP_NEFF", "1") == "1"):
             twin = self._second_lane()
diff --git a/include/gdhip.h b/include/gdhip.h
--- a/include/gdhip.h
+++ b/include/gdhip.h
@@ -409,6 +409,24 @@
 int gd_batch2d_invalidate(gd_ctx* ctx);
 int gd_batch2d_exchanges(gd_ctx* ctx, int64_t* count_out);
 
+typedef struct gd_prepared_param {
+    double range_min, range_max, sigma_range;
+    int32_t has_limits_bot, has_limits_top;
+} gd_prepared_param;
+
+typedef struct gd_prepare_settings {
+    int32_t fine_bins_2D;
+    int32_t auto_bandwidth;
+    int32_t uncorrelated_sampler;
+    int32_t ahead;
+} gd_prepare_settings;
+
+int gd_prepare_params(gd_ctx* ctx, gd_ctx* twin, const gd_prepare_settings* settings, const int32_t* cols, int32_t ncols,
+                      const double* targets, const double* minmax, const double* means, const double* vars, const double* err,
+                      const double* limits, double* quantiles_out, double* probe_out, int32_t* probe_done,
+                      gd_prepared_param* recs);
+int gd_prepare_ahead_counts(gd_ctx* ctx, int64_t* out3);
+
 
 int gd_comm_rccl_path(char* buf, int32_t len, int32_t* preloaded_out);
 int gd_upload_shard(gd_ctx* ctx, const double* X_cols, int64_t N, int64_t n, int64_t col_first, int64_t col_count,
```

Result: faster. 50970, median of 6 (+2.6%).
